# bifurcationkit/BifurcationKit.jl

Measured on AMD Instinct MI355X. Metric: newton_krylov_corrector_steps_per_s, higher is better.
Workload: dtype f64

## Files before the change

### bifurcationkit.jl_amd/_lib.py

```python
from __future__ import annotations

import ctypes as C
import os

_HERE = os.path.dirname(os.path.abspath(__file__))
LIB_PATH = os.environ.get("BKHIP_LIB") or os.path.join(_HERE, "lib", "libbkhip.so")

BK_ABI_VERSION = 6
BK_UNIQUE_ID_BYTES = 128
BK_MAX_PARAMS = 8
BK_MAX_NEWTON_ITER = 64

BK_PDE_SH, BK_PDE_SH1D, BK_PDE_CGL2D = 1, 2, 3
BK_GMRES_KRYLOVKIT, BK_GMRES_ITERATIVESOLVERS, BK_GMRES_KRYLOVJL = 0, 1, 2
BK_KRYLOV_MINRES, BK_KRYLOV_CG = 3, 4

c_double_p = C.POINTER(C.c_double)
c_int_p = C.POINTER(C.c_int)


class ProblemDesc(C.Structure):
    _fields_ = [("pde", C.c_int), ("ndim", C.c_int), ("n", C.c_int * 3), ("l", C.c_double * 3)]


# ... 96 lines not shown
    "bk_prof_enable": (I, [VP, I]),
    "bk_prof_reset": (I, [VP]),
    "bk_prof_get": (I, [VP, C.c_char_p, c_double_p, C.POINTER(C.c_longlong), c_double_p]),
    "bk_solver_history": (I, [VP, c_double_p, SZ, C.POINTER(SZ), I]),
    "bk_solver_block_log": (I, [VP, c_double_p, SZ, C.POINTER(SZ), I]),
    "bk_malloc": (I, [VP, SZ, C.POINTER(VP)]),
    "bk_free": (I, [VP, VP]),
    "bk_upload": (I, [VP, VP, c_double_p, SZ]),
    "bk_download": (I, [VP, c_double_p, VP, SZ]),
    "bk_vec_copy": (I, [VP, SZ, VP, VP]),
    "bk_vec_zero": (I, [VP, SZ, VP]),
    "bk_vec_scale": (I, [VP, SZ, D, VP]),
    "bk_vec_axpby": (I, [VP, SZ, D, VP, D, VP]),
    "bk_vec_dot": (I, [VP, SZ, VP, VP, c_double_p]),
    "bk_vec_nrm2": (I, [VP, SZ, VP, c_double_p]),
    "bk_vec_nrminf": (I, [VP, SZ, VP, c_double_p]),
    "bk_krylov_multidot": (I, [VP, SZ, VP, SZ, I, VP, c_double_p]),
    "bk_krylov_multiaxpy": (I, [VP, SZ, VP, SZ, I, c_double_p, VP, D, VP, c_double_p]),
    "bk_problem_create": (I, [VP, C.POINTER(ProblemDesc), C.POINTER(VP)]),
    "bk_problem_destroy": (I, [VP]),
    "bk_problem_nlocal": (I, [VP, C.POINTER(SZ), c_int_p, c_int_p]),
    "bk_residual": (I, [VP, VP, c_double_p, I, VP]),
    "bk_residual_dparam": (I, [VP, VP, c_double_p, I, I, D, VP]),
    "bk_jacobian": (I, [VP, VP, c_double_p, I, C.POINTER(VP)]),
    "bk_op_destroy": (I, [VP]),
    "bk_jacobian_adjoint": (I, [VP, VP, c_double_p, I, C.POINTER(VP)]),
    "bk_op_apply": (I, [VP, VP, D, D, VP]),
    "bk_precond_sh_create": (I, [VP, D, C.POINTER(VP)]),
    "bk_precond_lap_create": (I, [VP, D, C.POINTER(VP)]),
    "bk_precond_cgl_create": (I, [VP, D, D, C.POINTER(VP)]),
    "bk_precond_destroy": (I, [VP]),
    "bk_precond_apply": (I, [VP, VP, VP]),
    "bk_precond_op_apply": (I, [VP, VP, VP, VP, D, D, VP, c_int_p]),
    "bk_precond_check_norm": (I, [VP, VP, VP, VP, VP, D, D, I, c_double_p, c_int_p]),
    "bk_gmres_default_opts": (None, [C.POINTER(GmresOpts), I]),
    "bk_gmres": (I, [VP, VP, VP, VP, D, D, C.POINTER(GmresOpts), VP, c_int_p, c_int_p, c_double_p]),
    "bk_gmres2": (I, [VP, VP, VP, VP, VP, VP, D, D, C.POINTER(GmresOpts), VP, c_int_p, c_int_p]),
    "bk_palc_update": (I, [VP, SZ, D, VP, VP, VP]),
    "bk_bls_bordering": (I, [VP, VP, VP, VP, D, VP, D, D, D, I, D, D, C.POINTER(BorderingOpts),
                             C.POINTER(GmresOpts), VP, VP, c_double_p, c_int_p, c_int_p]),
    "bk_bls_matrixfree": (I, [VP, VP, VP, VP, D, VP, D, D, D, I, D, D, C.POINTER(GmresOpts), VP, c_double_p,
                              c_int_p, c_int_p]),
    "bk_bls_block_bordering": (I, [VP, VP, I, C.POINTER(VP), C.POINTER(VP), c_double_p, VP, c_double_p,
                                   C.POINTER(GmresOpts), VP, VP, c_double_p, c_int_p, c_int_p]),
    "bk_bls_block_matrixfree": (I, [VP, VP, I, C.POINTER(VP), C.POINTER(VP), c_double_p, VP, c_double_p, I, D, D,
                                    C.POINTER(GmresOpts), VP, c_double_p, c_int_p, c_int_p]),
    "bk_bls_matrixfree_pl": (I, [VP, VP, VP, VP, D, VP, D, D, D, I, D, D, C.POINTER(GmresOpts), VP, VP, c_double_p,
                                 c_int_p, c_int_p]),
    "bk_bls_block_matrixfree_pl": (I, [VP, VP, I, C.POINTER(VP), C.POINTER(VP), c_double_p, VP, c_double_p, I, D, D,
                                       C.POINTER(GmresOpts), VP, VP, c_double_p, c_int_p, c_int_p]),
    "bk_bordered_tail": (I, [VP, SZ, I, VP, VP, C.POINTER(VP), C.POINTER(VP), c_double_p, c_double_p]),
    "bk_gmres_cshift": (I, [VP, VP, VP, VP, VP, VP, D, D, D, C.POINTER(GmresOpts), VP, c_int_p, c_int_p, c_double_p]),
    "bk_bls_bordering_cshift": (I, [VP, VP, VP, VP, VP, VP, D, D, VP, VP, D, D, D, D, D, D, D, C.POINTER(GmresOpts),
                                    VP, VP, VP, c_double_p, c_int_p, c_int_p]),
    "bk_bls_matrixfree_pl_cshift": (I, [VP, VP, VP, VP, VP, VP, D, D, VP, VP, D, D, D, D, D, D, D, C.POINTER(GmresOpts),
                                        VP, VP, VP, c_double_p, c_int_p, c_int_p]),
    "bk_cbordered_tail": (I, [VP, SZ, VP, VP, VP, VP, VP, VP, VP, VP, c_double_p, c_double_p]),
    "bk_eig_shiftinvert": (I, [VP, VP, I, C.POINTER(EigOpts), C.POINTER(GmresOpts), VP, c_double_p, c_double_p,
                               VP, VP, SZ, c_int_p, c_int_p, c_int_p]),
    "bk_eig_set_start_vector": (I, [VP, VP]),
    "bk_eig_krylovkit": (I, [VP, VP, I, C.POINTER(EigOpts), c_double_p, c_double_p, VP, VP, SZ, c_int_p, c_int_p, c_int_p]),
    "bk_newton": (I, [VP, VP, VP, c_double_p, I, C.POINTER(NewtonOpts), C.POINTER(GmresOpts), VP,
                      C.POINTER(NewtonResult)]),
    "bk_cont_create": (I, [VP, VP, c_double_p, I, I, VP, D, VP, D, C.POINTER(ContOpts), C.POINTER(NewtonOpts),
                           C.POINTER(BorderingOpts), C.POINTER(GmresOpts), VP, C.POINTER(EigOpts),
                           C.POINTER(GmresOpts), VP, C.POINTER(ContStepResult), C.POINTER(VP)]),
    "bk_cont_step": (I, [VP, C.POINTER(ContStepResult)]),
    "bk_cont_get": (I, [VP, VP, c_double_p, VP, c_double_p, c_double_p]),
    "bk_cont_destroy": (I, [VP]),
    "bk_cont_clone": (I, [VP, C.POINTER(VP)]),
    "bk_cont_locate_bifurcation": (I, [VP, C.POINTER(BisectionOpts), C.POINTER(BisectionResult)]),
    "bk_newton_deflated": (I, [VP, VP, VP, c_double_p, I, C.POINTER(VP), I, D, D, I, D, C.POINTER(NewtonOpts),
                               C.POINTER(GmresOpts), VP, C.POINTER(NewtonResult)]),
    "bk_deflation_dots": (I, [VP, SZ, VP, VP, C.POINTER(VP), I, c_double_p, c_double_p]),
    "bk_newton_deflated_exact": (I, [VP, VP, VP, c_double_p, I, C.POINTER(VP), I, D, D, I, I, C.POINTER(NewtonOpts),
                                     C.POINTER(GmresOpts), VP, C.POINTER(DeflatedResult)]),
    "bk_deflation_dist": (I, [VP, SZ, VP, C.POINTER(VP), I, c_double_p, c_double_p]),
    "bk_vec_perturb": (I, [VP, SZ, VP, D, C.c_ulonglong, C.c_ulonglong]),
    "bk_defcont_seek": (I, [VP, VP, VP, c_double_p, I, C.POINTER(VP), I, D, D, I, I, I, D, I, C.POINTER(GmresOpts), VP,
                            c_double_p, I, C.POINTER(DefContSeekResult)]),
    "bk_newton_palc": (I, [VP, VP, VP, c_double_p, VP, D, VP, D, D, D, c_double_p, I, I, D, D,
                           C.POINTER(NewtonOpts), C.POINTER(BorderingOpts), C.POINTER(GmresOpts), VP,
                           C.POINTER(NewtonResult)]),
    "bk_d2f": (I, [VP, VP, c_double_p, I, VP, VP, VP]),
    "bk_djdp": (I, [VP, VP, c_double_p, I, I, VP, VP]),
    "bk_fold_contract": (I, [VP, VP, c_double_p, I, I, VP, VP, I, C.POINTER(VP), c_double_p]),
    "bk_fold_border": (I, [VP, VP, c_double_p, I, I, VP, VP, VP, c_double_p]),
    "bk_fold_terms": (I, [VP, VP, VP, c_double_p, I, I, VP, VP, C.POINTER(BorderingOpts), C.POINTER(GmresOpts), VP, VP, VP,
                          c_double_p, c_double_p, c_int_p, c_int_p]),
    "bk_fold_linsolve": (I, [VP, VP, VP, c_double_p, I, I, VP, VP, I, C.POINTER(VP), c_double_p, C.POINTER(GmresOpts), VP,
                             C.POINTER(VP), c_double_p, c_int_p, c_int_p]),
    "bk_newton_fold": (I, [VP, VP, VP, c_double_p, c_double_p, I, I, VP, VP, C.POINTER(NewtonOpts), C.POINTER(BorderingOpts),
                           C.POINTER(GmresOpts), VP, VP, VP, c_double_p, C.POINTER(NewtonResult)]),
    "bk_hopf_d2f": (I, [VP, VP, c_double_p, I, VP, VP, VP]),
    "bk_hopf_djdp": (I, [VP, VP, c_double_p, I, I, VP, VP]),
    "bk_hopf_contract": (I, [VP, VP, c_double_p, I, I, VP, VP, VP, VP, I, C.POINTER(VP), c_double_p]),
    "bk_hopf_terms": (I, [VP, VP, VP, c_double_p, I, I, D, VP, VP, VP, VP, C.POINTER(GmresOpts), VP, VP, VP, VP, VP,
                          c_double_p, c_double_p, c_double_p, c_int_p, c_int_p]),
    "bk_hopf_linsolve": (I, [VP, VP, VP, c_double_p, I, I, VP, VP, VP, VP, I, C.POINTER(VP), c_double_p, C.POINTER(GmresOpts),
                             VP, C.POINTER(VP), c_double_p, c_int_p, c_int_p]),
    "bk_newton_hopf": (I, [VP, VP, VP, c_double_p, c_double_p, c_double_p, I, I, VP, VP, VP, VP, C.POINTER(NewtonOpts),
                           C.POINTER(GmresOpts), VP, VP, VP, VP, VP, c_double_p, C.POINTER(NewtonResult)]),
    "bk_hopf_d3f": (I, [VP, VP, c_double_p, I, VP, VP, VP, VP]),
    "bk_hopf_nf_rhs": (I, [VP, VP, c_double_p, I, VP, VP, VP, VP, VP]),
    "bk_hopf_nf_contract": (I, [VP, VP, c_double_p, I, I, VP, VP, VP, VP, VP, VP, VP, VP, c_double_p]),
    "bk_hopf_normal_form": (I, [VP, VP, VP, c_double_p, I, I, D, VP, VP, VP, VP, C.POINTER(GmresOpts), VP, VP, VP, VP, VP,
                                c_double_p, c_int_p, c_int_p]),
    "bk_hopf_orbit": (I, [VP, SZ, VP, VP, VP, VP, VP, VP, VP, D, D, I, c_double_p, C.POINTER(VP)]),
    "bk_bautin_rhs3": (I, [VP, VP, c_double_p, I, VP, VP, VP, VP, VP, c_double_p, VP, VP, VP, VP]),
    "bk_bautin_rhs4": (I, [VP, VP, c_double_p, I, VP, VP, VP, VP, VP, VP, VP, VP, VP, c_double_p, VP, VP, VP]),
    "bk_bautin_contract": (I, [VP, VP, c_double_p, I, VP, VP, VP, VP, VP, VP, VP, VP, VP, VP, VP, VP, VP, VP, c_double_p]),
    "bk_bautin_normal_form": (I, [VP, VP, VP, c_double_p, I, D, VP, VP, VP, VP, VP, VP, VP, c_double_p, C.POINTER(GmresOpts), VP,
                                  VP, VP, VP, VP, VP, VP, VP, c_double_p, c_int_p, c_int_p]),
    "bk_d3f": (I, [VP, VP, c_double_p, I, VP, VP, VP, VP]),
    "bk_nf1d_dots": (I, [VP, VP, c_double_p, I, I, VP, VP, c_double_p]),
    "bk_nf1d_rhs": (I, [VP, VP, c_double_p, I, I, VP, D, D, VP, VP]),
    "bk_nf1d_contract": (I, [VP, VP, c_double_p, I, I, VP, VP, VP, VP, c_double_p]),
    "bk_nf1d_predict": (I, [VP, SZ, VP, VP, VP, VP, I, c_double_p, c_double_p, c_double_p, C.POINTER(VP)]),
    "bk_normal_form_1d": (I, [VP, VP, VP, c_double_p, I, I, VP, VP, C.POINTER(BorderingOpts), C.POINTER(GmresOpts), VP, VP, VP,
                              c_double_p, c_int_p, c_int_p]),
    "bk_cusp_dots": (I, [VP, VP, c_double_p, I, VP, VP, c_double_p]),
    "bk_cusp_rhs": (I, [VP, VP, c_double_p, I, VP, D, VP]),
    "bk_cusp_contract": (I, [VP, VP, c_double_p, I, VP, VP, VP, c_double_p]),
    "bk_cusp_normal_form": (I, [VP, VP, VP, c_double_p, I, VP, VP, C.POINTER(BorderingOpts), C.POINTER(GmresOpts), VP, VP,
                                c_double_p, c_int_p, c_int_p]),
    "bk_nfnd_dots": (I, [VP, VP, c_double_p, I, I, I, C.POINTER(VP), c_double_p]),
    "bk_nfnd_rhs": (I, [VP, VP, c_double_p, I, I, I, C.POINTER(VP), c_double_p, c_double_p, C.POINTER(VP)]),
    "bk_nfnd_contract": (I, [VP, VP, c_double_p, I, I, I, C.POINTER(VP), VP, C.POINTER(VP), c_double_p]),
    "bk_normal_form_nd": (I, [VP, VP, VP, c_double_p, I, I, I, C.POINTER(VP), C.POINTER(GmresOpts), VP, VP, C.POINTER(VP),
                              c_double_p, c_int_p, c_int_p]),
    "bk_potrap_create": (I, [VP, I, C.POINTER(VP)]),
    "bk_potrap_destroy": (I, [VP]),
    "bk_potrap_set_section": (I, [VP, VP, VP]),
    "bk_potrap_residual": (I, [VP, VP, D, c_double_p, I, VP, c_double_p]),
    "bk_potrap_jvp": (I, [VP, VP, D, c_double_p, I, VP, D, VP, c_double_p]),
    "bk_potrap_op_create": (I, [VP, VP, D, c_double_p, I, C.POINTER(VP)]),
    "bk_potrap_update_section": (I, [VP, VP, D, c_double_p, I]),
    "bk_potrap_dparam": (I, [VP, VP, D, c_double_p, I, I, VP]),
    "bk_precond_potrap_create": (I, [VP, D, D, C.POINTER(VP)]),
    "bk_precond_potrap_set_period": (I, [VP, D]),
    "bk_precond_potrap_transform_paths": (I, [VP, c_int_p]),
    "bk_potrap_get_section": (I, [VP, VP, VP]),
    "bk_potrap_solve": (I, [VP, VP, VP, VP, D, VP, c_double_p, C.POINTER(GmresOpts), C.POINTER(SolveResult)]),
    "bk_potrap_jvp_adjoint": (I, [VP, VP, D, c_double_p, I, VP, D, VP, c_double_p]),
    "bk_potrap_op_adjoint_create": (I, [VP, VP, D, c_double_p, I, C.POINTER(VP)]),
    "bk_precond_potrap_adjoint_create": (I, [VP, D, D, C.POINTER(VP)]),
    "bk_potrap_bordered_solve": (I, [VP, VP, VP, VP, D, VP, D, D, VP, D, D, VP, c_double_p, c_double_p, C.POINTER(GmresOpts),
                                     C.POINTER(SolveResult)]),
    "bk_potrap_fold_border": (I, [VP, VP, D, c_double_p, I, I, VP, D, VP, VP, c_double_p, c_double_p]),
    "bk_potrap_fold_terms": (I, [VP, VP, D, c_double_p, I, VP, D, VP, D, VP, VP, C.POINTER(GmresOpts), VP, c_double_p, VP,
                                 c_double_p, c_double_p, c_int_p, c_int_p]),
    "bk_potrap_fold_linsolve": (I, [VP, VP, D, c_double_p, I, I, VP, D, VP, VP, I, C.POINTER(VP), c_double_p, c_double_p,
                                    C.POINTER(GmresOpts), C.POINTER(VP), c_double_p, c_double_p, c_int_p, c_int_p]),
    "bk_potrap_newton_fold": (I, [VP, VP, c_double_p, c_double_p, c_double_p, I, I, VP, D, VP, D, VP, VP, C.POINTER(NewtonOpts),
                                  C.POINTER(GmresOpts), VP, c_double_p, VP, c_double_p, c_double_p, C.POINTER(NewtonResult),
                                  c_int_p]),
    "bk_potrap_ivp_march": (I, [VP, VP, D, c_double_p, I, VP, VP]),
    "bk_precond_potrap_ivp_create": (I, [VP, D, D, D, C.POINTER(VP)]),
    "bk_precond_potrap_ivp_transform_paths": (I, [VP, c_int_p]),
    "bk_potrap_monodromy_create": (I, [VP, VP, D, c_double_p, I, D, D, C.POINTER(GmresOpts), C.POINTER(VP)]),
    "bk_potrap_monodromy_solve": (I, [VP, VP, VP, c_int_p, c_int_p]),
    "bk_potrap_monodromy_stats": (I, [VP, c_int_p, c_int_p, c_int_p, c_int_p]),
    "bk_eig_krylovkit_lm": (I, [VP, VP, I, C.POINTER(EigOpts), c_double_p, c_double_p, VP, VP, SZ, c_int_p, c_int_p, c_int_p]),
}

_lib = None
# ... 38 lines not shown
```

### bifurcationkit.jl_amd/csrc/common.h

```cpp
#pragma once

#include <hip/hip_runtime.h>
#include <rccl/rccl.h>

#include <cstdarg>
#include <cstdio>
#include <cstring>
#include <map>
#include <set>
#include <string>
#include <utility>
#include <vector>

#include "../../include/bkhip.h"

namespace bk {

constexpr int kMaxBasis = 64;
constexpr int kRedSlots = 256;
constexpr int kRedBlocks = 1024;
constexpr int kPartialVals = 72;
constexpr size_t kPartialDoubles = (size_t)kRedBlocks * kPartialVals;
constexpr double kCancelTol = 1e-8;
constexpr int kRecChunks = 16;
// ... 98 lines not shown
namespace bk {

int set_error(bk_ctx* ctx, const char* fmt, ...);

#define BK_HIP(ctx, call)                                                                     \
    do {                                                                                      \
        hipError_t e_ = (call);                                                               \
        if (e_ != hipSuccess)                                                                 \
            return bk::set_error((ctx), "%s:%d: %s failed: %s", __FILE__, __LINE__, #call,    \
                                 hipGetErrorString(e_));                                      \
    } while (0)

#define BK_NCCL(ctx, call)                                                                    \
    do {                                                                                      \
        ncclResult_t e_ = (call);                                                             \
        if (e_ != ncclSuccess)                                                                \
            return bk::set_error((ctx), "%s:%d: %s failed: %s", __FILE__, __LINE__, #call,    \
                                 ncclGetErrorString(e_));                                     \
    } while (0)

#define BK_TRY(call)             \
    do {                         \
        int s_ = (call);         \
        if (s_ != 0) return s_;  \
    } while (0)

bk_ctx* ctx_lane(bk_ctx* ctx);
void ctx_lane_merge(bk_ctx* ctx, bk_ctx* lane);

int ws_get(bk_ctx* ctx, size_t n, double** out);
void ws_put(bk_ctx* ctx, double* p);

struct WsGuard {
    bk_ctx* ctx;
    std::vector<double*> ptrs;
    explicit WsGuard(bk_ctx* c) : ctx(c) {}
    ~WsGuard() { for (double* p : ptrs) ws_put(ctx, p); }
    int get(size_t n, double** out) {
        int s = ws_get(ctx, n, out);
        if (s == 0) ptrs.push_back(*out);
        return s;
    }
};

struct ProfScope {
    bk_ctx* ctx;
    ProfEntry* e = nullptr;
    hipEvent_t start = nullptr, stop = nullptr;
    ProfScope(bk_ctx* c, const char* name, double alg_bytes);
    ~ProfScope();
};

int reduce_finish(bk_ctx* ctx, int nblocks, int nvals, int op);
int comm_allreduce_host(bk_ctx* ctx, double* buf, int n, int op);
int comm_allreduce_dev(bk_ctx* ctx, hipStream_t stream, double* dbuf, int n, int op);
int ctx_sync(bk_ctx* ctx);
void proxy_destroy(bk_ctx* ctx);

void blas_release(bk_ctx* ctx);
int v_copy(bk_ctx* ctx, size_t n, const double* x, double* y);
int v_zero(bk_ctx* ctx, size_t n, double* x);
int v_scale(bk_ctx* ctx, size_t n, double a, double* x);
int v_axpby(bk_ctx* ctx, size_t n, double a, const double* x, double b, double* y);
int v_axpbyz(bk_ctx* ctx, size_t n, double a, const double* x, double b, const double* y, double* z);
int v_pw_scale(bk_ctx* ctx, size_t n, const double* x, const double* u, double A, double B, double C, double* z);
int v_dot(bk_ctx* ctx, size_t n, const double* x, const double* y, double* out);
int v_dot2(bk_ctx* ctx, size_t n, const double* x, const double* y1, const double* y2, double* out2);
int v_nrm2(bk_ctx* ctx, size_t n, const double* x, double* out);
int v_diff_nrm2(bk_ctx* ctx, size_t n, const double* x, const double* y, double* out);
int v_axpy_dot(bk_ctx* ctx, size_t n, double c, const double* r, double* y, const double* z, double* out);
int v_minres_update(bk_ctx* ctx, size_t n, double cz, const double* z, double c1, const double* w1, double c2, const double* w2,
                    double* w, double phi, double* x);
int v_minres_update2(bk_ctx* ctx, size_t n, double cza, const double* za, double c1a, double c2a, double czb, const double* zb, double c1b,
                     double c2b, const double* m2, const double* m1, double* wa, double* wb, double phia, double phib, double* x);
int v_nrminf(bk_ctx* ctx, size_t n, const double* x, double* out);
int v_multidot(bk_ctx* ctx, size_t n, const double* V, size_t ldv, int k, const double* w, double* out);
bool v_multidot_gram_ok(bk_ctx* ctx, size_t n, const double* V, size_t ldv, int k, const double* w);
int v_multidot_gram(bk_ctx* ctx, size_t n, const double* V, size_t ldv, int k, const double* w, double* out, double* gram);
int v_multiaxpy(bk_ctx* ctx, size_t n, const double* V, size_t ldv, int k, const double* c,
                const double* src, double scale, double* dst, double* nrm2sq);
bool v_block_ok(bk_ctx* ctx, size_t n, const double* V, size_t ldv);
int v_block_dots(bk_ctx* ctx, size_t n, const double* V, size_t ldv, int kold, int r0, int nr, double* D, double* T);
int v_block_axpy(bk_ctx* ctx, size_t n, double* V, size_t ldv, int k, int s, const double* Cm, const double* Tm);
int v_arnoldi_step_dev(bk_ctx* ctx, size_t n, double* V, size_t ldv, int k, const double* w, double eta, double orth_tol,
                       double* rec, double* coef, double* gram = nullptr);
int v_basis_combine(bk_ctx* ctx, size_t n, const double* V, size_t ldv, int m, const double* Qhost, int kout,
                    double* dst, size_t lddst);
int v_fill_random(bk_ctx* ctx, size_t n, size_t global_offset, unsigned long long seed, double* x);

}
```

### bifurcationkit.jl_amd/csrc/cont.hip

```cpp
#include <cmath>
#include <vector>

#include "ops.h"

using namespace bk;

struct bk_cont {
    bk_ctx* ctx = nullptr;
    bk_problem* prob = nullptr;
    size_t n = 0;
    double Nglob = 1.0;
    double params[BK_MAX_PARAMS];
    int nparams = 0, ipar = 0;
    bk_cont_opts co;
    bk_newton_opts no;
    bk_bordering_opts bo;
    bk_gmres_opts lo;
    bk_precond* pl = nullptr;
    bool has_eig = false;
    bk_eig_opts eo;
    bk_gmres_opts elo;
    bk_precond* epl = nullptr;
    double *zu = nullptr, *zoldu = nullptr, *tauu = nullptr, *predu = nullptr, *work = nullptr, *work2 = nullptr;
    double zp = 0, zoldp = 0, taup = 0, predp = 0, ds = 0;
// ... 100 lines not shown
        if (r->vals_re[i] > c->co.tol_stability) {
            ++nu;
            if (std::fabs(r->vals_im[i]) > c->co.tol_stability) ++ni;
        }
    }
    r->nvals = nvals;
    r->eig_converged = nconv >= nev;
    r->eig_numops = nops;
    c->n_unstable_prev = c->n_unstable;
    c->n_imag_prev = c->n_imag;
    c->n_unstable = nu;
    c->n_imag = ni;
    c->nvals = nvals;
    for (int i = 0; i < nvals; ++i) { c->vals_re[i] = r->vals_re[i]; c->vals_im[i] = r->vals_im[i]; }
    return 0;
}

}

extern "C" {

int bk_cont_create(bk_ctx* ctx, bk_problem* prob, const double* params, int nparams, int ipar, const double* u0,
                   double p0, const double* u1, double p1, const bk_cont_opts* copts, const bk_newton_opts* nopts,
                   const bk_bordering_opts* bopts, const bk_gmres_opts* lsopts, bk_precond* pl,
                   const bk_eig_opts* eopts, const bk_gmres_opts* eig_lsopts, bk_precond* eig_pl,
                   bk_cont_step_result* init, bk_cont** out) {
    if (!ctx || !prob || !params || !u0 || !u1 || !copts || !nopts || !bopts || !lsopts || !out) return -1;
    if (ipar < 0 || ipar >= nparams || nparams > BK_MAX_PARAMS) return set_error(ctx, "bad parameter index");
    if (copts->detect && (!eopts || !eig_lsopts)) return set_error(ctx, "bk_cont_create: detect needs eigensolver options");
    if (nopts->max_iterations > BK_MAX_NEWTON_ITER) return set_error(ctx, "max_iterations > %d", BK_MAX_NEWTON_ITER);
    bk_cont* c = new bk_cont();
    c->ctx = ctx; c->prob = prob; c->n = prob->nloc;
    for (int a = 0; a < prob->desc.ndim; ++a) c->Nglob *= prob->desc.n[a];
    if (prob->desc.pde == BK_PDE_CGL2D) c->Nglob *= 2.0;
    for (int i = 0; i < BK_MAX_PARAMS; ++i) c->params[i] = i < nparams ? params[i] : 0.0;
    c->nparams = nparams; c->ipar = ipar;
    c->co = *copts; c->no = *nopts; c->bo = *bopts; c->lo = *lsopts; c->pl = pl;
    c->has_eig = copts->detect != 0;
    if (c->has_eig) { c->eo = *eopts; c->elo = *eig_lsopts; c->epl = eig_pl; }
    c->thick = c->has_eig && ctx->opt("eig_thick_start", 0.0) != 0.0;
    double** bufs[] = {&c->zu, &c->zoldu, &c->tauu, &c->predu, &c->work, &c->work2, &c->eigx0};
    for (double** b : bufs) {
        if (b == &c->eigx0 && !c->thick) continue;
        if (hipMalloc(b, c->n * sizeof(double)) != hipSuccess) {
            bk_cont_destroy(c);
            return set_error(ctx, "bk_cont_create: device allocation failed");
        }
    }
    int s = 0;
    c->ds = copts->ds;
    if ((s = v_copy(ctx, c->n, u0, c->zu)) || (s = v_copy(ctx, c->n, u0, c->zoldu))) { bk_cont_destroy(c); return s; }
    c->zp = c->zoldp = p0;
    bk_cont_step_result r0 = {};
    r0.converged = 1; r0.p = p0; r0.ds_used = c->ds; r0.n_unstable = -1; r0.n_imag = -1;
    if (c->has_eig && (s = eigen(c, &r0))) { bk_cont_destroy(c); return s; }
    r0.n_unstable = c->n_unstable; r0.n_imag = c->n_imag;
    if ((s = secant_tangent(c, u1, p1, u0, p0, c->ds)) || (s = predictor(c))) { bk_cont_destroy(c); return s; }
    r0.ds_next = c->ds;
    if (init) *init = r0;
    *out = c;
    return 0;
}

int bk_cont_destroy(bk_cont* c) {
    if (!c) return 0;
    double* bufs[] = {c->zu, c->zoldu, c->tauu, c->predu, c->work, c->work2, c->eigx0};
    for (double* b : bufs)
        if (b) (void)hipFree(b);
    delete c;
    return 0;
}

int bk_cont_step(bk_cont* c, bk_cont_step_result* r) {
    if (!c || !r) return -1;
    bk_ctx* ctx = c->ctx;
    *r = bk_cont_step_result{};
    r->n_unstable = c->n_unstable; r->n_imag = c->n_imag;
    r->p = c->zp; r->ds_used = c->ds; r->ds_next = c->ds;
    if (c->step > 0 && !(c->zp > c->co.p_min && c->zp < c->co.p_max)) {
        r->stop = 2;
        return 0;
    }
    double* x = c->work;
    BK_TRY(v_copy(ctx, c->n, c->predu, x));
    double p = c->predp;
    bk_newton_result nr = {};
    if (c->predp <= c->co.p_min || c->predp >= c->co.p_max) {
        c->predp = p = std::min(std::max(c->predp, c->co.p_min), c->co.p_max);
        double par[BK_MAX_PARAMS];
        for (int i = 0; i < c->nparams; ++i) par[i] = c->params[i];
        par[c->ipar] = p;
        BK_TRY(bk_newton(ctx, c->prob, x, par, c->nparams, &c->no, &c->lo, c->pl, &nr));
        r->natural = 1;
    } else {
        BK_TRY(bk_newton_palc(ctx, c->prob, x, &p, c->zu, c->zp, c->tauu, c->taup, c->ds, c->co.theta, c->params,
                              c->nparams, c->ipar, c->co.p_min, c->co.p_max, &c->no, &c->bo, &c->lo, c->pl, &nr));
    }
    r->converged = nr.converged; r->itnewton = nr.itnewton; r->itlinear = nr.itlinear;
    c->converged = nr.converged != 0;
    for (int i = 0; i <= nr.itnewton && i <= BK_MAX_NEWTON_ITER; ++i) r->residuals[i] = nr.residuals[i];
    const int prev_unst = c->n_unstable;
    if (nr.converged) {
        BK_TRY(v_copy(ctx, c->n, c->zu, c->zoldu));
        c->zoldp = c->zp;
        BK_TRY(v_copy(ctx, c->n, x, c->zu));
        c->zp = p;
        if (c->has_eig) {
            BK_TRY(eigen(c, r));
            if (prev_unst != -1 && c->n_unstable != prev_unst) r->bifurcation = 1;
        }
        c->step += 1;
    }
    r->p = c->zp;
    r->n_unstable = c->n_unstable; r->n_imag = c->n_imag;
    r->step = c->step;
    double ds = c->ds;
    if (!c->stepsizecontrol) {
    } else if (!nr.converged) {
        if (std::fabs(ds) <= c->co.dsmin) {
            r->stop = 1;
            return 0;
        }
        ds = std::copysign(std::max(std::fabs(ds) / 2.0, c->co.dsmin), ds);
    } else {
        const double Nmax = c->no.max_iterations;
        const double factor = (Nmax - nr.itnewton) / Nmax;
        ds = ds * (1.0 + c->co.a * factor * factor);
    }
    if (c->stepsizecontrol)
        ds = std::copysign(std::min(std::max(std::fabs(ds), c->co.dsmin), c->co.dsmax), ds);
    c->ds = ds;
    r->ds_next = ds;
    if (nr.converged) {
        if (c->co.tangent == 0) {
            BK_TRY(secant_tangent(c, c->zu, c->zp, c->zoldu, c->zoldp, ds));
            r->tangent_converged = 1;
        } else {
            BK_TRY(bordered_tangent(c, &r->tangent_converged));
        }
    }
    BK_TRY(predictor(c));
    return 0;
}

static int cont_copy_state(bk_cont* dst, const bk_cont* src) {
    double* d[] = {dst->zu, dst->zoldu, dst->tauu, dst->predu};
    const double* from[] = {src->zu, src->zoldu, src->tauu, src->predu};
    for (int i = 0; i < 4; ++i) BK_TRY(v_copy(src->ctx, src->n, from[i], d[i]));
    dst->zp = src->zp; dst->zoldp = src->zoldp; dst->taup = src->taup; dst->predp = src->predp; dst->ds = src->ds;
    dst->n_unstable = src->n_unstable; dst->n_imag = src->n_imag; dst->step = src->step;
    dst->n_unstable_prev = src->n_unstable_prev; dst->n_imag_prev = src->n_imag_prev;
    dst->stepsizecontrol = src->stepsizecontrol; dst->converged = src->converged;
    dst->nvals = src->nvals;
    for (int i = 0; i < src->nvals; ++i) { dst->vals_re[i] = src->vals_re[i]; dst->vals_im[i] = src->vals_im[i]; }
    if (src->thick && dst->thick && src->have_x0) BK_TRY(v_copy(src->ctx, src->n, src->eigx0, dst->eigx0));
    dst->have_x0 = src->thick && dst->thick && src->have_x0;
    return 0;
}

int bk_cont_clone(bk_cont* src, bk_cont** out) {
    if (!src || !out) return -1;
    bk_cont* c = new bk_cont(*src);
    c->zu = c->zoldu = c->tauu = c->predu = c->work = c->work2 = c->eigx0 = nullptr;
    double** bufs[] = {&c->zu, &c->zoldu, &c->tauu, &c->predu, &c->work, &c->work2, &c->eigx0};
    for (double** b : bufs) {
        if (b == &c->eigx0 && !c->thick) continue;
        if (hipMalloc(b, c->n * sizeof(double)) != hipSuccess) {
            bk_cont_destroy(c);
            return set_error(src->ctx, "bk_cont_clone: device allocation failed");
        }
    }
    const int s = cont_copy_state(c, src);
    if (s != 0) { bk_cont_destroy(c); return s; }
    *out = c;
    return 0;
}

int bk_cont_locate_bifurcation(bk_cont* c, const bk_bisection_opts* bo, bk_bisection_result* res) {
    if (!c || !bo || !res) return -1;
// ... 193 lines not shown
```

### bifurcationkit.jl_amd/csrc/ops.h

```cpp
#pragma once

#include "common.h"

namespace bk {

int halo_exchange(bk_ctx* ctx, hipStream_t stream, const double* v, size_t plane, int nplanes, int width, double* halo_lo,
                  double* halo_hi);

int comm_alltoallv(bk_ctx* ctx, const double* sendbuf, const size_t* scount, const size_t* sdispl, double* recvbuf,
                   const size_t* rcount, const size_t* rdispl);

struct ShArgs {
    int nx, ny, nz;
    int nzg, zoff;
    double ax, ay, az;
    double l, nu;
    double a0, a1;
    double ag = 0.0;
    bool ag_set = false;
    int mode;
    const double* v;
    const double* u;
    double* out;
    const double* halo_lo;
// ... 93 lines not shown
                     double* out, double* dot, int* fused);
    int dparam(const double* u, const double* params, int nparams, int ipar, double eps, const double* f0, double* out);
};

struct bk_op {
    bk_ctx* ctx = nullptr;
    size_t n = 0;
    int ntail = 0;
    virtual ~bk_op() {}
    virtual int apply(const double* x, const double* xt, double a0, double a1, double* out, double* outt) = 0;
    virtual int apply_axpy_dot(const double* x, double a0, double a1, double c, const double* r, double* out, double* dot);
    virtual bool shift_is_free() const { return false; }
    virtual int apply_block(const double* x, int s, double a0, double a1, const double* theta, double* const* outs) {
        for (int i = 0; i < s; ++i) {
            const int e = apply(i == 0 ? x : outs[i - 1], nullptr, a0 - (theta ? theta[i] : 0.0), a1, outs[i], nullptr);
            if (e != 0) return e;
        }
        return 0;
    }
    virtual int apply_parts(const double* x, double a0, double aL, double ag, double* out) { return 1; }
    virtual const bk_problem* sh_problem() const { return nullptr; }
    virtual bool sh_state(const double** u, double* l, double* nu) const { return false; }
    virtual int apply_check(const double* x, const double* xt, double a0, double a1, double* out, double* outt) {
        return apply(x, xt, a0, a1, out, outt);
    }
    virtual int check_norm(const double* x, double a0, double a1, double* nrm, int* done) { *done = 0; return 0; }
    virtual int apply_check_resume(const double* x, double a0, double a1, double* out) { return apply_check(x, nullptr, a0, a1, out, nullptr); }
    virtual bool hessenberg_shift() const { return false; }
    virtual double monomial_shift() const { return 0.0; }
    virtual double rearranged_origin() const { return 0.0; }
    virtual bool arm_v0(const double* src, double scale, double* dst) { return false; }
    virtual void disarm_v0() {}
};

struct bk_precond {
    bk_ctx* ctx = nullptr;
    size_t n = 0;
    virtual ~bk_precond() {}
    virtual int apply(const double* v, double* out) = 0;
    virtual int apply_dot(const double* v, double* out, double* dot);
    virtual int apply_dot_pre_axpy(double* y, double c, const double* r, double* out, double* dot);
    virtual int apply_nrm2(const double* v, double c, const double* add, double* nrm2_out, bool store_sum = true);
    virtual bool nrm2_spectral_ok() const { return false; }
    virtual bool is_l1_plus_shift(const bk_problem* prob, double* shift) const { return false; }
    virtual int apply_pw(const double* x, const bk::DctFuse& d, double cx, double ct, double* out);
    int pw_src_first(bk::DctFuse& d);
    virtual bool pw_fused_ok(const double* x, const double* u, const double* out) const { return false; }
    virtual int apply_pw_chain(const double* x, const bk::DctFuse& d, int s, const double* cx, double ct, double* const* outs);
    virtual bool pw_plan_ok() const { return false; }
    int pw_agreed = -1;
};

namespace bk {

struct PdeJacobian : bk_op {
    bk_problem* prob;
    const double* u;
    double params[BK_MAX_PARAMS];
    bool adjoint = false;
    int apply(const double* x, const double* xt, double a0, double a1, double* out, double* outt) override;
    int apply_axpy_dot(const double* x, double a0, double a1, double c, const double* r, double* out, double* dot) override;
    bool shift_is_free() const override { return true; }
    int apply_parts(const double* x, double a0, double aL, double ag, double* out) override;
    const bk_problem* sh_problem() const override;
    bool sh_state(const double** u_, double* l, double* nu) const override;
};

bk_precond* precond_lane_shadow(bk_precond* pl, bk_ctx* lane);

struct GmresResult {
    int converged = 0;
    int niter = 0;
    double resnorm = 0.0;
};
int gmres_core(bk_ctx* ctx, bk_op* A, const double* b, const double* bt, double* x, double* xt, double alpha0,
               double alpha1, const bk_gmres_opts& o, GmresResult* res);
int linsolve(bk_ctx* ctx, bk_op* J, const double* rhs, double* x, double a0, double a1, const bk_gmres_opts& o,
             bk_precond* pl, GmresResult* res);
int linsolve2(bk_ctx* ctx, bk_op* J, const double* rhs1, double* x1, const double* rhs2, double* x2, double a0, double a1,
              const bk_gmres_opts& o, bk_precond* pl, GmresResult* r1, GmresResult* r2);
int bls_bordering(bk_ctx* ctx, bk_op* J, const double* dR, const double* dzu, double dzp, const double* R, double nn,
                  double xiu, double xip, bool has_shift, double shift, double dotscale, const bk_bordering_opts& bo,
                  const bk_gmres_opts& ls, bk_precond* pl, double* dX, double* dl, int* converged, int itlinear[2],
                  double* xnew = nullptr);
struct PrecOpView {
    bk_op* op = nullptr;
    bool tmode = false;
    double alpha0 = 0.0, alpha1 = 1.0;
};
int prec_op_create(bk_ctx* ctx, bk_op* J, bk_precond* pl, double a0, double a1, int order, double* tmp, PrecOpView* out);
int bls_matrixfree_pl(bk_ctx* ctx, bk_op* J, int m, const double* const* a, const double* const* b, double bscale, const double* c,
                      const double* rhst, const double* rhsb, bool has_shift, double shift, const bk_gmres_opts& ls, bk_precond* pl,
                      double* u1, double* u2, GmresResult* res, const double* const* atil = nullptr);
int cshift_op_create(bk_ctx* ctx, bk_op* J, bk_precond* pl, double a0r, double a0i, double a1, int order, double* tmp, bk_op** out);
int bordered_tail(bk_ctx* ctx, size_t n, int m, double* y, const double* x, const double* const* atil, const double* const* b,
                  const double* coef, double* dots);
int cbordered_tail(bk_ctx* ctx, size_t n, double* yr, double* yi, const double* xr, const double* xi, const double* atr,
                   const double* ati, const double* br, const double* bi, const double* coef, double* dots);
int bls_matrixfree_pl_cshift(bk_ctx* ctx, bk_op* J, const double* const a[2], const double* const b[2], double bscale, const double c[2],
                             const double* const rhst[2], const double rhsb[2], const double shift[2], const bk_gmres_opts& ls,
                             bk_precond* pl, double* u1_re, double* u1_im, double u2[2], GmresResult* res);
int newton_cb(const bk_newton_opts* no, const double* x, const double* fx, double residual, int step, int itlinear, double p,
              const double* z0u, double z0p, int from_newton);

}
```

### bifurcationkit.jl_amd/csrc/solver.hip

```cpp
#include <cmath>
#include <cstdio>
#include <thread>
#include <vector>

#include "dense.h"
#include "ops.h"
#include "sstep.h"
#include "stream.h"

namespace bk {

namespace {

constexpr double kCheckSpectralDefault = 1.0;

constexpr double kMonomialShiftDefault = 0.0;

inline size_t round_up(size_t n, size_t m) { return (n + m - 1) / m * m; }

struct Basis {
    double* V = nullptr;
    size_t ld = 0;
    int nt = 0;
    double dlt = 0.0;
// ... 1007 lines not shown
        o->dim = 30; o->maxiter = 100; o->atol = 1e-12; o->rtol = 1e-12;
    }
}

int bk_gmres(bk_ctx* ctx, bk_op* J, const double* rhs, double* x, double a0, double a1, const bk_gmres_opts* opts,
             bk_precond* pl, int* converged, int* niter, double* resnorm) {
    if (!ctx || !J || !rhs || !x || !opts) return -1;
    GmresResult r;
    BK_TRY(linsolve(ctx, J, rhs, x, a0, a1, *opts, pl, &r));
    if (converged) *converged = r.converged;
    if (niter) *niter = r.niter;
    if (resnorm) *resnorm = r.resnorm;
    return 0;
}

int bk_precond_op_apply(bk_ctx* ctx, bk_precond* pl, bk_op* J, const double* x, double a0, double a1, double* out, int* stencil_free) {
    if (!ctx || !pl || !J || !x || !out) return -1;
    if (J->ntail != 0) return set_error(ctx, "bk_precond_op_apply: operator must be unbordered");
    if (out == x) return set_error(ctx, "bk_precond_op_apply: out must not alias x");
    WsGuard ws(ctx);
    ShiftPrecOp W;
    W.ctx = ctx; W.n = J->n; W.ntail = 0;
    W.J = J; W.P = pl; W.a0 = a0; W.a1 = a1; W.order = 0; W.tmp = nullptr;
    BK_TRY(W.init_fold());
    BK_TRY(ws.get(J->n, &W.tmp));
    if (stencil_free) *stencil_free = W.tmode ? 1 : 0;
    return W.tmode ? W.apply(x, nullptr, W.t_alpha0, W.t_alpha1, out, nullptr) : W.apply(x, nullptr, 0.0, 1.0, out, nullptr);
}

int bk_precond_check_norm(bk_ctx* ctx, bk_precond* pl, bk_op* J, const double* x, const double* rhs, double a0, double a1, int flavor,
                          double* nrm, int* spectral) {
    if (!ctx || !pl || !J || !x || !rhs || !nrm) return -1;
    if (J->ntail != 0) return set_error(ctx, "bk_precond_check_norm: operator must be unbordered");
    if (flavor != BK_GMRES_KRYLOVKIT && flavor != BK_GMRES_ITERATIVESOLVERS && flavor != BK_GMRES_KRYLOVJL)
        return set_error(ctx, "bk_precond_check_norm: a GMRES flavor");
    WsGuard ws(ctx);
    ShiftPrecOp W;
    W.ctx = ctx; W.n = J->n; W.ntail = 0;
    W.J = J; W.P = pl; W.a0 = a0; W.a1 = a1; W.order = flavor == BK_GMRES_KRYLOVKIT ? 0 : 1; W.tmp = nullptr;
    BK_TRY(W.init_fold());
    W.rhs = rhs;
    BK_TRY(ws.get(J->n, &W.tmp));
    const double alpha0 = W.tmode ? W.t_alpha0 : 0.0, alpha1 = W.tmode ? W.t_alpha1 : 1.0;
    int have = 0;
    BK_TRY(W.check_norm(x, alpha0, alpha1, nrm, &have));
    if (spectral) *spectral = have;
    if (have) return 0;
    double *b = nullptr, *w = nullptr;
    BK_TRY(ws.get(J->n, &b));
    BK_TRY(ws.get(J->n, &w));
    BK_TRY(pl->apply(rhs, b));
    BK_TRY(W.apply_check(x, nullptr, alpha0, alpha1, w, nullptr));
    return v_diff_nrm2(ctx, J->n, b, w, nrm);
}

int bk_abi_version(void) { return BK_ABI_VERSION; }

int bk_gmres2(bk_ctx* ctx, bk_op* J, const double* rhs1, const double* rhs2, double* x1, double* x2, double a0,
              double a1, const bk_gmres_opts* opts, bk_precond* pl, int* converged, int niter[2]) {
    if (!ctx || !J || !rhs1 || !rhs2 || !x1 || !x2 || !opts) return -1;
    if (x1 == x2) return set_error(ctx, "bk_gmres2: x1 and x2 must be distinct buffers");
    GmresResult r1, r2;
    BK_TRY(linsolve2(ctx, J, rhs1, x1, rhs2, x2, a0, a1, *opts, pl, &r1, &r2));
    if (converged) *converged = r1.converged & r2.converged;
    if (niter) { niter[0] = r1.niter; niter[1] = r2.niter; }
    return 0;
}

}

namespace bk {

struct BorderingState {
    double* dx = nullptr;
    bool have_dx = false;
    int it_dx = 0;
    int cv_dx = 1;
};

namespace {

template <int VEC, bool NTH>
__global__ void __launch_bounds__(kThreads) palc_update_kernel(size_t n, double a, const double* __restrict__ dx,
                                                               const double* __restrict__ x1, double* x, int has_dx) {
    auto one = [&](double d, double v, double xv) {
        double t = 0.0;
        if (has_dx) t = __dmul_rn(a, d);
        t = __dadd_rn(t, v);
        return __dadd_rn(-t, xv);
    };
    if (VEC == 2) {
        stream_loop<4>(n >> 1, [&](auto uc, size_t i0, size_t st) {
            constexpr int UU = decltype(uc)::value;
            double2 dv[UU], vv[UU], xv[UU];
#pragma unroll
            for (int u = 0; u < UU; ++u) {
                dv[u] = ld2<NTH>(dx, i0 + u * st);
                vv[u] = ld2<NTH>(x1, i0 + u * st);
                xv[u] = ld2<NTH>(x, i0 + u * st);
            }
#pragma unroll
            for (int u = 0; u < UU; ++u) {
                const double rx = one(dv[u].x, vv[u].x, xv[u].x), ry = one(dv[u].y, vv[u].y, xv[u].y);
                if (NTH) {
                    nt_d2 r; r.x = rx; r.y = ry;
                    __builtin_nontemporal_store(r, reinterpret_cast<nt_d2*>(x) + (i0 + u * st));
                } else {
                    reinterpret_cast<double2*>(x)[i0 + u * st] = make_double2(rx, ry);
                }
            }
        });
        if ((n & 1) && blockIdx.x == 0 && threadIdx.x == 0) x[n - 1] = one(dx[n - 1], x1[n - 1], x[n - 1]);
    } else {
        for (size_t i = (size_t)blockIdx.x * kThreads + threadIdx.x; i < n; i += (size_t)gridDim.x * kThreads) x[i] = one(dx[i], x1[i], x[i]);
    }
}

}

int palc_update(bk_ctx* ctx, size_t n, double dl, const double* dx, const double* x1, double* x) {
    if (n == 0) return 0;
    ProfScope ps(ctx, "blas1", 32.0 * n);
    const bool vec = aligned16(dx) && aligned16(x1) && aligned16(x);
    const int grid = grid_for(n, vec ? 2 : 1, 4096);
    const double a = -dl;
    const int has_dx = a != 0.0 ? 1 : 0;
    if (vec && nt_hint(ctx, n))
        hipLaunchKernelGGL((palc_update_kernel<2, true>), dim3(grid), dim3(kThreads), 0, ctx->stream, n, a, dx, x1, x, has_dx);
    else if (vec)
        hipLaunchKernelGGL((palc_update_kernel<2, false>), dim3(grid), dim3(kThreads), 0, ctx->stream, n, a, dx, x1, x, has_dx);
    else
        hipLaunchKernelGGL((palc_update_kernel<1, false>), dim3(grid), dim3(kThreads), 0, ctx->stream, n, a, dx, x1, x, has_dx);
    BK_HIP(ctx, hipGetLastError());
    return 0;
}

static int bec(bk_ctx* ctx, bk_op* J, const double* dR, const double* dzu, double dzp, const double* R, double nn,
               double xiu, double xip, bool has_shift, double shift, double dotscale, const bk_gmres_opts& ls,
               bk_precond* pl, BorderingState& st, double* x1, double* dl, int* cv, int it[2], double* xnew = nullptr) {
    const size_t n = J->n;
    GmresResult r1;
    const double a0 = has_shift ? shift : 0.0;
    if (!st.have_dx) {
        GmresResult r2;
        BK_TRY(linsolve2(ctx, J, R, x1, dR, st.dx, a0, 1.0, ls, pl, &r1, &r2));
        st.have_dx = true; st.it_dx = r2.niter; st.cv_dx = r2.converged;
    } else {
        BK_TRY(linsolve(ctx, J, R, x1, a0, 1.0, ls, pl, &r1));
    }
    double d[2];
    BK_TRY(v_dot2(ctx, n, dzu, x1, st.dx, d));
    d[0] *= dotscale; d[1] *= dotscale;
    *dl = (nn - d[0] * xiu) / (dzp * xip - d[1] * xiu);
    if (xnew) BK_TRY(palc_update(ctx, n, *dl, st.dx, x1, xnew));
    else BK_TRY(v_axpby(ctx, n, -(*dl), st.dx, 1.0, x1));
    *cv = r1.converged & st.cv_dx;
    it[0] = r1.niter; it[1] = st.it_dx;
    return 0;
}

int bls_bordering(bk_ctx* ctx, bk_op* J, const double* dR, const double* dzu, double dzp, const double* R, double nn,
                  double xiu, double xip, bool has_shift, double shift, double dotscale, const bk_bordering_opts& bo,
                  const bk_gmres_opts& ls, bk_precond* pl, double* dX, double* dl, int* converged, int itlinear[2],
                  double* xnew) {
    if (xnew && bo.check_precision) return set_error(ctx, "bls_bordering: the fused update needs check_precision off");
    const size_t n = J->n;
    WsGuard ws(ctx);
    BorderingState st;
    BK_TRY(ws.get(n, &st.dx));
    int cv = 0, it[2] = {0, 0};
    BK_TRY(bec(ctx, J, dR, dzu, dzp, R, nn, xiu, xip, has_shift, shift, dotscale, ls, pl, st, dX, dl, &cv, it, xnew));
    int k = 0;
    bool fail = true;
    double *dXr = nullptr, *dX1 = nullptr;
    while (bo.check_precision && k < bo.k && fail) {
        if (!dXr) { BK_TRY(ws.get(n, &dXr)); BK_TRY(ws.get(n, &dX1)); }
        BK_TRY(J->apply(dX, nullptr, has_shift ? shift : 0.0, 1.0, dXr, nullptr));
        BK_TRY(v_axpby(ctx, n, *dl, dR, 1.0, dXr));
        BK_TRY(v_axpby(ctx, n, 1.0, R, -1.0, dXr));
        double dd, nr;
        BK_TRY(v_dot(ctx, n, dzu, dX, &dd));
        const double dlr = nn - xip * dzp * (*dl) - xiu * dotscale * dd;
        BK_TRY(v_nrm2(ctx, n, dXr, &nr));
        fail = nr > bo.tol || std::fabs(dlr) > bo.tol;
        if (fail) {
            double dl1 = 0.0;
            BK_TRY(bec(ctx, J, dR, dzu, dzp, dXr, dlr, xiu, xip, has_shift, shift, dotscale, ls, pl, st, dX1, &dl1, &cv, it));
            BK_TRY(v_axpby(ctx, n, 1.0, dX1, 1.0, dX));
            *dl += dl1;
            k += 1;
        }
    }
    if (converged) *converged = cv;
    if (itlinear) { itlinear[0] = it[0]; itlinear[1] = it[1]; }
    return 0;
}

struct BorderedMapOp : bk_op {
    bk_op* J;
    const double* a[BK_MAX_BORDER];
    const double* bvec[BK_MAX_BORDER];
    double bscale;
    double c[BK_MAX_BORDER * BK_MAX_BORDER];
    bool has_shift;
    double shift;
    int apply(const double* x, const double* xt, double b0, double b1, double* out, double* outt) override {
        const int m = ntail;
        BK_TRY(J->apply(x, nullptr, b0 + b1 * (has_shift ? shift : 0.0), b1, out, nullptr));
        for (int i = 0; i < m; ++i)
            if (xt[i] != 0.0 && b1 != 0.0) BK_TRY(v_axpby(ctx, n, b1 * xt[i], a[i], 1.0, out));
        for (int i = 0; i < m; ++i) {
            double d;
            BK_TRY(v_dot(ctx, n, bvec[i], x, &d));
            double cx = 0.0;
            for (int j = 0; j < m; ++j) cx += c[i * m + j] * xt[j];
            outt[i] = b0 * xt[i] + b1 * (bscale * d + cx);
        }
        return 0;
    }
};

int bls_matrixfree(bk_ctx* ctx, bk_op* J, const double* dR, const double* dzu, double dzp, const double* R, double n, double xiu,
                   double xip, bool has_shift, double shift, double dotscale, const bk_gmres_opts& ls, double* dX, double* dl,
                   int* converged, int* itlinear) {
    if (ls.flavor >= BK_KRYLOV_MINRES) return set_error(ctx, "bk_bls_matrixfree: the bordered operator is not symmetric (use a GMRES flavor)");
    BorderedMapOp M;
    M.ctx = ctx; M.n = J->n; M.ntail = 1;
    M.J = J; M.a[0] = dR; M.bvec[0] = dzu; M.bscale = xiu * dotscale; M.c[0] = dzp * xip;
    M.has_shift = has_shift; M.shift = shift;
    GmresResult r;
    BK_TRY(gmres_core(ctx, &M, R, &n, dX, dl, 0.0, 1.0, ls, &r));
    if (converged) *converged = r.converged;
    if (itlinear) *itlinear = r.niter;
    return 0;
}

}

extern "C" {

int bk_bls_bordering(bk_ctx* ctx, bk_op* J, const double* dR, const double* dzu, double dzp, const double* R,
                     double n, double xiu, double xip, int has_shift, double shift, double dotscale,
                     const bk_bordering_opts* bopts, const bk_gmres_opts* lsopts, bk_precond* pl, double* dX,
                     double* dl, int* converged, int itlinear[2]) {
    if (!ctx || !J || !dR || !dzu || !R || !bopts || !lsopts || !dX || !dl) return -1;
    if (dX == R || dX == dR || dX == dzu) return set_error(ctx, "bk_bls_bordering: dX must be a fresh buffer");
    if (bopts->k < 1) return set_error(ctx, "BorderingBLS: number of recursions must be positive");
    return bls_bordering(ctx, J, dR, dzu, dzp, R, n, xiu, xip, has_shift != 0, shift, dotscale, *bopts, *lsopts, pl, dX,
                         dl, converged, itlinear);
}

int bk_palc_update(bk_ctx* ctx, size_t n, double dl, const double* dx, const double* x1, double* x) {
    if (!ctx || !dx || !x1 || !x) return -1;
    if (x == dx || x == x1) return set_error(ctx, "bk_palc_update: x must not alias dx or x1");
    return palc_update(ctx, n, dl, dx, x1, x);
}

int bk_bls_matrixfree(bk_ctx* ctx, bk_op* J, const double* dR, const double* dzu, double dzp, const double* R,
                      double n, double xiu, double xip, int has_shift, double shift, double dotscale,
                      const bk_gmres_opts* lsopts, double* dX, double* dl, int* converged, int* itlinear) {
    if (!ctx || !J || !dR || !dzu || !R || !lsopts || !dX || !dl) return -1;
    if (dX == R || dX == dR || dX == dzu) return set_error(ctx, "bk_bls_matrixfree: dX must be a fresh buffer");
    return bls_matrixfree(ctx, J, dR, dzu, dzp, R, n, xiu, xip, has_shift != 0, shift, dotscale, *lsopts, dX, dl, converged, itlinear);
}

int bk_bls_block_bordering(bk_ctx* ctx, bk_op* J, int m, const double* const* b, const double* const* c, const double* d,
                           const double* rhst, const double* rhsb, const bk_gmres_opts* lsopts, bk_precond* pl,
                           double* u1, double* u2, int* converged, int* itlinear) {
    if (!ctx || !J || !b || !c || !d || !rhst || !rhsb || !lsopts || !u1 || !u2) return -1;
    if (m < 1 || m > BK_MAX_BORDER) return set_error(ctx, "Linear bordered solver, wrong sizes! (1 <= m <= %d)", BK_MAX_BORDER);
    if (u1 == rhst) return set_error(ctx, "bk_bls_block_bordering: u1 must be a fresh buffer");
    const size_t n = J->n;
    WsGuard ws(ctx);
    double* x2[BK_MAX_BORDER];
    GmresResult g;
    BK_TRY(linsolve(ctx, J, rhst, u1, 0.0, 1.0, *lsopts, pl, &g));
    int cv = 1;
    for (int j = 0; j < m; ++j) {
        if (!b[j] || !c[j]) return -1;
        BK_TRY(ws.get(n, &x2[j]));
        BK_TRY(linsolve(ctx, J, b[j], x2[j], 0.0, 1.0, *lsopts, pl, &g));
        cv &= g.converged;
        if (itlinear) itlinear[j] = g.niter;
    }
    double S[BK_MAX_BORDER][BK_MAX_BORDER + 1];
    for (int i = 0; i < m; ++i) {
        double t;
        for (int j = 0; j < m; ++j) {
            BK_TRY(v_dot(ctx, n, c[i], x2[j], &t));
            S[i][j] = d[i * m + j] - t;
        }
        BK_TRY(v_dot(ctx, n, c[i], u1, &t));
        S[i][m] = rhsb[i] - t;
    }
    for (int k = 0; k < m; ++k) {
        int piv = k;
        for (int i = k + 1; i < m; ++i)
            if (std::fabs(S[i][k]) > std::fabs(S[piv][k])) piv = i;
        if (S[piv][k] == 0.0) return set_error(ctx, "bk_bls_block_bordering: singular Schur complement");
        if (piv != k)
            for (int j = 0; j <= m; ++j) std::swap(S[k][j], S[piv][j]);
        for (int i = k + 1; i < m; ++i) {
            const double f = S[i][k] / S[k][k];
            for (int j = k; j <= m; ++j) S[i][j] -= f * S[k][j];
        }
    }
    for (int i = m - 1; i >= 0; --i) {
        double t = S[i][m];
        for (int j = i + 1; j < m; ++j) t -= S[i][j] * u2[j];
        u2[i] = t / S[i][i];
    }
    for (int j = 0; j < m; ++j) BK_TRY(v_axpby(ctx, n, -u2[j], x2[j], 1.0, u1));
    if (converged) *converged = cv;
    return 0;
}

int bk_bls_block_matrixfree(bk_ctx* ctx, bk_op* J, int m, const double* const* a, const double* const* b, const double* c,
                            const double* rhst, const double* rhsb, int has_shift, double shift, double dotscale,
                            const bk_gmres_opts* lsopts, double* u1, double* u2, int* converged, int* itlinear) {
    if (!ctx || !J || !a || !b || !c || !rhst || !rhsb || !lsopts || !u1 || !u2) return -1;
    if (m < 1 || m > BK_MAX_BORDER) return set_error(ctx, "Linear bordered solver, wrong sizes! (1 <= m <= %d)", BK_MAX_BORDER);
    if (u1 == rhst) return set_error(ctx, "bk_bls_block_matrixfree: u1 must be a fresh buffer");
    if (lsopts->flavor >= BK_KRYLOV_MINRES) return set_error(ctx, "bk_bls_block_matrixfree: the bordered operator is not symmetric (use a GMRES flavor)");
    BorderedMapOp M;
    M.ctx = ctx; M.n = J->n; M.ntail = m;
    M.J = J; M.bscale = dotscale;
    for (int i = 0; i < m; ++i) {
        if (!a[i] || !b[i]) return -1;
        M.a[i] = a[i]; M.bvec[i] = b[i];
        for (int j = 0; j < m; ++j) M.c[i * m + j] = c[i * m + j];
    }
    M.has_shift = has_shift != 0; M.shift = shift;
    GmresResult r;
    BK_TRY(gmres_core(ctx, &M, rhst, rhsb, u1, u2, 0.0, 1.0, *lsopts, &r));
    if (converged) *converged = r.converged;
    if (itlinear) *itlinear = r.niter;
    return 0;
}

}

namespace bk {

static int norm_of(bk_ctx* ctx, size_t n, const double* x, bool inf, double* out) {
    return inf ? v_nrminf(ctx, n, x, out) : v_nrm2(ctx, n, x, out);
}

int newton_cb(const bk_newton_opts* no, const double* x, const double* fx, double residual, int step, int itlinear,
              double p, const double* z0u, double z0p, int from_newton) {
    if (no->max_residual > 0.0 && !(residual < no->max_residual)) return 0;
    if (no->callback) return no->callback(no->callback_user, x, fx, residual, step, itlinear, p, z0u, z0p, from_newton) != 0;
    return 1;
}

}

extern "C" {

int bk_newton(bk_ctx* ctx, bk_problem* prob, double* x, const double* params, int nparams, const bk_newton_opts* no,
              const bk_gmres_opts* lsopts, bk_precond* pl, bk_newton_result* res) {
    if (!ctx || !prob || !x || !params || !no || !lsopts || !res) return -1;
    if (no->max_iterations > BK_MAX_NEWTON_ITER) return set_error(ctx, "max_iterations > %d", BK_MAX_NEWTON_ITER);
    const size_t n = prob->nloc;
    WsGuard ws(ctx);
    double *fx = nullptr, *u = nullptr;
    BK_TRY(ws.get(n, &fx));
    BK_TRY(ws.get(n, &u));
    BK_TRY(bk_residual(prob, x, params, nparams, fx));
    double r;
    BK_TRY(norm_of(ctx, n, fx, no->norm_inf != 0, &r));
    int step = 0, itlin = 0;
    res->residuals[0] = r;
    int compute = newton_cb(no, x, fx, r, 0, 0, NAN, nullptr, NAN, 1);
    while (step < no->max_iterations && r > no->tol && compute) {
        bk_op* J = nullptr;
        BK_TRY(bk_jacobian(prob, x, params, nparams, &J));
        GmresResult g;
        int s = linsolve(ctx, J, fx, u, 0.0, 1.0, *lsopts, pl, &g);
        bk_op_destroy(J);
        if (s != 0) return s;
        itlin += g.niter;
        BK_TRY(v_axpby(ctx, n, -1.0, u, 1.0, x));
        BK_TRY(bk_residual(prob, x, params, nparams, fx));
        BK_TRY(norm_of(ctx, n, fx, no->norm_inf != 0, &r));
        step += 1;
        res->residuals[step] = r;
        compute = newton_cb(no, x, fx, r, step, g.niter, NAN, nullptr, NAN, 1);
    }
    res->converged = (res->residuals[step] < no->tol) & newton_cb(no, x, fx, r, step, 0, NAN, nullptr, NAN, 1);
    res->itnewton = step;
    res->itlinear = itlin;
    return 0;
}

int bk_newton_palc(bk_ctx* ctx, bk_problem* prob, double* x, double* p, const double* z0u, double z0p,
                   const double* tauu, double taup, double ds, double theta, const double* params, int nparams,
                   int ipar, double p_min, double p_max, const bk_newton_opts* no, const bk_bordering_opts* bo,
                   const bk_gmres_opts* lsopts, bk_precond* pl, bk_newton_result* res) {
    if (!ctx || !prob || !x || !p || !z0u || !tauu || !params || !no || !bo || !lsopts || !res) return -1;
    if (ipar < 0 || ipar >= nparams || nparams > BK_MAX_PARAMS) return set_error(ctx, "bad parameter index");
    if (no->max_iterations > BK_MAX_NEWTON_ITER) return set_error(ctx, "max_iterations > %d", BK_MAX_NEWTON_ITER);
    const size_t n = prob->nloc;
    double Nglob = 1.0;
    for (int a = 0; a < prob->desc.ndim; ++a) Nglob *= prob->desc.n[a];
    if (prob->desc.pde == BK_PDE_CGL2D) Nglob *= 2.0;
    const double dotscale = 1.0 / Nglob;
    const double eps = 1.4901161193847656e-08;
    WsGuard ws(ctx);
    double *res_f = nullptr, *dFdp = nullptr, *u = nullptr, *x_pred = nullptr;
    BK_TRY(ws.get(n, &res_f));
    BK_TRY(ws.get(n, &dFdp));
    BK_TRY(ws.get(n, &u));
    const bool linesearch = no->linesearch != 0;
    if (linesearch) BK_TRY(ws.get(n, &x_pred));
    const double alpha0 = no->alpha > 0.0 ? no->alpha : 1.0;
    const double alpha_min = no->alpha_min > 0.0 ? no->alpha_min : 1e-3;
    double alpha = alpha0;
    double par[BK_MAX_PARAMS];
    for (int i = 0; i < nparams; ++i) par[i] = params[i];
    const bool inf = no->norm_inf != 0;
    double dz0;
    BK_TRY(v_dot(ctx, n, z0u, tauu, &dz0));
    auto Nfun = [&](const double* xx, double pp, double* out) -> int {
        double d;
        BK_TRY(v_dot(ctx, n, xx, tauu, &d));
        *out = (d * dotscale * theta + (pp - z0p) * taup * (1.0 - theta) - ds) - (dz0 * dotscale * theta);
        return 0;
    };
    double pc = *p;
    par[ipar] = pc;
    BK_TRY(bk_residual(prob, x, par, nparams, res_f));
    double res_n, rf;
    BK_TRY(Nfun(x, pc, &res_n));
    BK_TRY(norm_of(ctx, n, res_f, inf, &rf));
    double r = std::max(rf, std::fabs(res_n));
    int step = 0, itlin = 0;
    res->residuals[0] = r;
    bool line_step = true;
    const bool fuse_update = bo->kind == 0 && bo->check_precision == 0 && !linesearch && ctx->opt("palc_fuse_update", 1.0) != 0.0;
    int compute = newton_cb(no, x, res_f, r, 0, 0, pc, z0u, z0p, 0);
    while (step < no->max_iterations && r > no->tol && line_step && compute) {
        par[ipar] = pc;
        BK_TRY(prob->dparam(x, par, nparams, ipar, eps, res_f, dFdp));
        bk_op* J = nullptr;
        BK_TRY(bk_jacobian(prob, x, par, nparams, &J));
        double up = 0.0;
        int cv = 0, it[2] = {0, 0};
        int s;
        if (bo->kind == 1) {
            int itm = 0;
            s = bls_matrixfree(ctx, J, dFdp, tauu, taup, res_f, res_n, theta, 1.0 - theta, false, 0.0, dotscale, *lsopts, u, &up, &cv, &itm);
            it[0] = itm; it[1] = 0;
        } else {
            s = bls_bordering(ctx, J, dFdp, tauu, taup, res_f, res_n, theta, 1.0 - theta, false, 0.0, dotscale, *bo,
                              *lsopts, pl, u, &up, &cv, it, fuse_update ? x : nullptr);
        }
        bk_op_destroy(J);
        if (s != 0) return s;
        itlin += it[0] + it[1];
        if (linesearch) {
            line_step = false;
            while (!line_step && alpha > alpha_min) {
                BK_TRY(v_axpbyz(ctx, n, 1.0, x, -alpha, u, x_pred));
                const double p_pred = pc - alpha * up;
                par[ipar] = p_pred;
                BK_TRY(bk_residual(prob, x_pred, par, nparams, res_f));
                BK_TRY(Nfun(x_pred, p_pred, &res_n));
                BK_TRY(norm_of(ctx, n, res_f, inf, &rf));
                r = std::max(rf, std::fabs(res_n));
                if (r < res->residuals[step]) {
                    if (r < res->residuals[step] / 4.0 && alpha < 1.0) alpha *= 2.0;
                    line_step = true;
                    BK_TRY(v_copy(ctx, n, x_pred, x));
                    pc = std::min(std::max(p_pred, p_min), p_max);
                } else {
                    alpha /= 2.0;
                }
            }
            alpha = alpha0;
            par[ipar] = pc;
        } else {
            if (!fuse_update) BK_TRY(v_axpby(ctx, n, -1.0, u, 1.0, x));
            pc = std::min(std::max(pc - up, p_min), p_max);
            par[ipar] = pc;
            BK_TRY(bk_residual(prob, x, par, nparams, res_f));
            BK_TRY(Nfun(x, pc, &res_n));
            BK_TRY(norm_of(ctx, n, res_f, inf, &rf));
            r = std::max(rf, std::fabs(res_n));
        }
        step += 1;
        res->residuals[step] = r;
        compute = newton_cb(no, x, res_f, r, step, it[0] + it[1], pc, z0u, z0p, 0);
    }
    *p = pc;
    res->converged = (res->residuals[step] < no->tol) & newton_cb(no, x, res_f, r, step, 0, pc, z0u, z0p, 0);
    res->itnewton = step;
    res->itlinear = itlin;
    return 0;
}

}
```

### bifurcationkit.jl_amd/csrc/vecops.hip

```cpp
#include <algorithm>
#include <type_traits>

#include "common.h"
#include "sstep.h"
#include "stream.h"

namespace bk {

namespace {

struct StreamRange { size_t lo, hi, step; };
__device__ __forceinline__ StreamRange stream_range(size_t n2, unsigned xcd) {
    StreamRange r;
    if (xcd) {
        const size_t x = blockIdx.x & 7u, lb = blockIdx.x >> 3, nb = gridDim.x >> 3;
        const size_t per = ((n2 + 7) / 8 + kThreads - 1) / kThreads * kThreads;
        const size_t b0 = x * per < n2 ? x * per : n2, b1 = (x + 1) * per < n2 ? (x + 1) * per : n2;
        r.lo = b0 + lb * kThreads + threadIdx.x; r.hi = b1; r.step = nb * kThreads;
    } else {
        r.lo = (size_t)blockIdx.x * kThreads + threadIdx.x; r.hi = n2; r.step = (size_t)gridDim.x * kThreads;
    }
    return r;
}

inline unsigned xcd_map(bk_ctx* ctx, size_t n, int grid, bool axpy, int k) {
    const int mode = (int)ctx->opt("vec_xcd_map", 1.0);
    if (!(nt_hint(ctx, n) && grid >= 8 && grid % 8 == 0) || mode == 0) return 0u;
    return (mode >= 2 || (axpy && k >= 12)) ? 1u : 0u;
}

__device__ __forceinline__ double max_nan(double a, double b) { return (a != a || a > b) ? a : b; }
__device__ __forceinline__ double wave_max(double v) {
#pragma unroll
    for (int off = 32; off > 0; off >>= 1) v = max_nan(v, __shfl_down(v, off, 64));
    return v;
}

__device__ __forceinline__ void st2nt(double* p, size_t i, double2 v) {
    nt_d2 r; r.x = v.x; r.y = v.y;
    __builtin_nontemporal_store(r, reinterpret_cast<nt_d2*>(p) + i);
}


template <int VEC, bool NTH = false>
__global__ void __launch_bounds__(kThreads) axpbyz_kernel(size_t n, double a, const double* __restrict__ x, double b,
                                                          const double* y, double* z, int has_x, int has_y) {
    const size_t stride = (size_t)gridDim.x * kThreads;
    if (VEC == 2) {
        const size_t n2 = n >> 1;
        auto run = [&](auto hx, auto hy) {
            constexpr bool HX = decltype(hx)::value, HY = decltype(hy)::value;
            stream_loop<4>(n2, [&](auto uc, size_t i0, size_t st) {
                constexpr int UU = decltype(uc)::value;
                double2 xv[UU], yv[UU];
#pragma unroll
                for (int u = 0; u < UU; ++u) {
                    if (HX) xv[u] = ld2<NTH>(x, i0 + u * st);
                    if (HY) yv[u] = ld2<NTH>(y, i0 + u * st);
                }
#pragma unroll
                for (int u = 0; u < UU; ++u) {
                    double2 r = make_double2(0.0, 0.0);
                    if (HX) { r.x = a * xv[u].x; r.y = a * xv[u].y; }
                    if (HY) { r.x += b * yv[u].x; r.y += b * yv[u].y; }
                    if (NTH) st2nt(z, i0 + u * st, r);
                    else reinterpret_cast<double2*>(z)[i0 + u * st] = r;
                }
            });
        };
        if (has_x && has_y) run(std::true_type{}, std::true_type{});
        else if (has_x) run(std::true_type{}, std::false_type{});
        else if (has_y) run(std::false_type{}, std::true_type{});
        else run(std::false_type{}, std::false_type{});
        if ((n & 1) && blockIdx.x == 0 && threadIdx.x == 0) {
            const size_t i = n - 1;
            double r = 0.0;
            if (has_x) r = a * x[i];
            if (has_y) r += b * y[i];
            z[i] = r;
        }
    } else {
        for (size_t i = (size_t)blockIdx.x * kThreads + threadIdx.x; i < n; i += stride) {
            double r = 0.0;
            if (has_x) r = a * x[i];
            if (has_y) r += b * y[i];
// ... 115 lines not shown
            stream_loop<2>(n2, [&](auto uc, size_t i0, size_t st) {
                constexpr int UU = decltype(uc)::value;
                double2 yv[UU], rv[UU], zv[UU];
#pragma unroll
                for (int u = 0; u < UU; ++u) {
                    yv[u] = ld2<NTH>(y, i0 + u * st);
                    if (HR) rv[u] = ld2<NTH>(r, i0 + u * st);
                    zv[u] = ld2<NTH>(z, i0 + u * st);
                }
#pragma unroll
                for (int u = 0; u < UU; ++u) {
                    if (HR) {
                        yv[u].x = fma(c, rv[u].x, yv[u].x); yv[u].y = fma(c, rv[u].y, yv[u].y);
                        if (NTH) st2nt(y, i0 + u * st, yv[u]);
                        else reinterpret_cast<double2*>(y)[i0 + u * st] = yv[u];
                    }
                    s = fma(zv[u].x, yv[u].x, s); s = fma(zv[u].y, yv[u].y, s);
                }
            });
        };
        if (has_r) run(std::true_type{}); else run(std::false_type{});
        if ((n & 1) && blockIdx.x == 0 && threadIdx.x == 0) {
            double yv = y[n - 1];
            if (has_r) { yv = fma(c, r[n - 1], yv); y[n - 1] = yv; }
            s = fma(z[n - 1], yv, s);
        }
    } else {
        for (size_t i = (size_t)blockIdx.x * kThreads + threadIdx.x; i < n; i += stride) {
            double yv = y[i];
            if (has_r) { yv = fma(c, r[i], yv); y[i] = yv; }
            s = fma(z[i], yv, s);
        }
    }
    __shared__ double sm[4];
    s = wave_sum(s);
    if ((threadIdx.x & 63) == 0) sm[threadIdx.x >> 6] = s;
    __syncthreads();
    if (threadIdx.x == 0) partials[blockIdx.x] = (sm[0] + sm[1]) + (sm[2] + sm[3]);
}

template <int VEC, bool NTH = false>
__global__ void __launch_bounds__(kThreads) minres_update_kernel(size_t n, double cz, const double* __restrict__ z, double c1,
                                                                 const double* __restrict__ w1, double c2,
                                                                 const double* __restrict__ w2, double* __restrict__ w,
                                                                 double phi, double* __restrict__ x) {
    const size_t stride = (size_t)gridDim.x * kThreads;
    if (VEC == 2) {
        const size_t n2 = n >> 1;
        stream_loop<2>(n2, [&](auto uc, size_t i0, size_t st) {
            constexpr int UU = decltype(uc)::value;
            double2 zv[UU], a[UU], b[UU], xv[UU];
#pragma unroll
            for (int u = 0; u < UU; ++u) {
                zv[u] = ld2<NTH>(z, i0 + u * st);
                a[u] = ld2<NTH>(w1, i0 + u * st);
                b[u] = ld2<NTH>(w2, i0 + u * st);
                xv[u] = ld2<NTH>(x, i0 + u * st);
            }
#pragma unroll
            for (int u = 0; u < UU; ++u) {
                double2 wv;
                wv.x = fma(c2, b[u].x, fma(c1, a[u].x, cz * zv[u].x));
                wv.y = fma(c2, b[u].y, fma(c1, a[u].y, cz * zv[u].y));
                xv[u].x = fma(phi, wv.x, xv[u].x); xv[u].y = fma(phi, wv.y, xv[u].y);
                if (NTH) { st2nt(w, i0 + u * st, wv); st2nt(x, i0 + u * st, xv[u]); }
                else { reinterpret_cast<double2*>(w)[i0 + u * st] = wv; reinterpret_cast<double2*>(x)[i0 + u * st] = xv[u]; }
            }
        });
        if ((n & 1) && blockIdx.x == 0 && threadIdx.x == 0) {
            const size_t i = n - 1;
            const double wv = fma(c2, w2[i], fma(c1, w1[i], cz * z[i]));
            w[i] = wv;
            x[i] = fma(phi, wv, x[i]);
        }
    } else {
        for (size_t i = (size_t)blockIdx.x * kThreads + threadIdx.x; i < n; i += stride) {
            const double wv = fma(c2, w2[i], fma(c1, w1[i], cz * z[i]));
            w[i] = wv;
            x[i] = fma(phi, wv, x[i]);
        }
    }
}

__global__ void __launch_bounds__(kThreads) absmax_kernel(size_t n, const double* __restrict__ x,
                                                          double* __restrict__ partials) {
    const size_t stride = (size_t)gridDim.x * kThreads;
    double m = 0.0;
    for (size_t i = (size_t)blockIdx.x * kThreads + threadIdx.x; i < n; i += stride) m = max_nan(m, fabs(x[i]));
    __shared__ double sm[4];
    m = wave_max(m);
    if ((threadIdx.x & 63) == 0) sm[threadIdx.x >> 6] = m;
    __syncthreads();
    if (threadIdx.x == 0) partials[blockIdx.x] = max_nan(max_nan(sm[0], sm[1]), max_nan(sm[2], sm[3]));
}

template <int KB, int VEC, bool LDNT = false>
__global__ void __launch_bounds__(kThreads) multidot_kernel(size_t n, const double* __restrict__ V, size_t ldv, int k,
                                                            const double* __restrict__ w,
                                                            double* __restrict__ partials, const double* gate = nullptr,
                                                            unsigned xcd = 0) {
    if (gate && gate[0] == 0.0) return;
    double acc[KB];
#pragma unroll
    for (int j = 0; j < KB; ++j) acc[j] = 0.0;
    double ww = 0.0;
    const size_t stride = (size_t)gridDim.x * kThreads;
    if (VEC == 2) {
        const StreamRange rg = stream_range(n >> 1, xcd);
        for (size_t i = rg.lo; i < rg.hi; i += rg.step) {
            const double2 wv = ld2<LDNT>(w, i);
            ww = fma(wv.x, wv.x, ww); ww = fma(wv.y, wv.y, ww);
#pragma unroll
            for (int j = 0; j < KB; ++j) {
                if (j < k) {
                    const double2 vv = ld2<LDNT>(V + (size_t)j * ldv, i);
                    acc[j] = fma(vv.x, wv.x, acc[j]);
                    acc[j] = fma(vv.y, wv.y, acc[j]);
                }
            }
        }
        if ((n & 1) && blockIdx.x == 0 && threadIdx.x == 0) {
            const double wv = w[n - 1];
            ww = fma(wv, wv, ww);
#pragma unroll
            for (int j = 0; j < KB; ++j)
                if (j < k) acc[j] = fma(V[(size_t)j * ldv + n - 1], wv, acc[j]);
        }
    } else {
        for (size_t i = (size_t)blockIdx.x * kThreads + threadIdx.x; i < n; i += stride) {
            const double wv = w[i];
            ww = fma(wv, wv, ww);
#pragma unroll
            for (int j = 0; j < KB; ++j)
                if (j < k) acc[j] = fma(V[(size_t)j * ldv + i], wv, acc[j]);
        }
    }
    __shared__ double sm[4][KB + 1];
    const int lane = threadIdx.x & 63, wid = threadIdx.x >> 6;
#pragma unroll
    for (int j = 0; j < KB; ++j) {
        const double s = wave_sum(acc[j]);
        if (lane == 0) sm[wid][j] = s;
    }
    {
        const double s = wave_sum(ww);
        if (lane == 0) sm[wid][KB] = s;
    }
    __syncthreads();
    for (int j = threadIdx.x; j <= k; j += kThreads) {
        const int src = (j == k) ? KB : j;
        partials[(size_t)blockIdx.x * (k + 1) + j] = (sm[0][src] + sm[1][src]) + (sm[2][src] + sm[3][src]);
    }
}

template <int KB, int VEC, bool NT = false, bool LDNT = false, int U = 1, bool DEV = false>
__global__ void __launch_bounds__(kThreads) multiaxpy_kernel(size_t n, const double* __restrict__ V, size_t ldv, int k,
                                                             Coefs cf, const double* src, double scale, double* dst,
                                                             int want_norm, double* __restrict__ partials, unsigned xcd = 0,
                                                             const double* __restrict__ dcoef = nullptr, int gated = 0) {
    if (DEV) {
        if (gated && dcoef[kMaxBasis + 1] == 0.0) return;
        scale = dcoef[kMaxBasis];
#pragma unroll
        for (int j = 0; j < KB; ++j) cf.c[j] = j < k ? dcoef[j] : 0.0;
    }
    double nn = 0.0;
    if (VEC == 2) {
        const StreamRange rg = stream_range(n >> 1, xcd);
        const size_t n2 = rg.hi, stride = rg.step;
        for (size_t i0 = rg.lo; i0 < n2; i0 += stride * U) {
            double2 r[U];
// ... 125 lines not shown
    }
    {
        const double s_ = wave_sum(ww);
        if (lane == 0) sm[wid][KB] = s_;
    }
    if (GRAM) {
#pragma unroll
        for (int j = 0; j < KB; ++j) {
            const double s_ = wave_sum(accg[j]);
            if (lane == 0) sm[wid][KB + 1 + j] = s_;
        }
    }
    __syncthreads();
    const int nv = GRAM ? 2 * k + 1 : k + 1;
    for (int j = threadIdx.x; j < nv; j += kThreads) {
        const int src = j < k ? j : (j == k ? KB : KB + 1 + (j - k - 1));
        partials[(size_t)blockIdx.x * nv + j] = (sm[0][src] + sm[1][src]) + (sm[2][src] + sm[3][src]);
    }
}

template <int KB, int U, bool NT, bool LDNT, bool DEV>
__global__ void __launch_bounds__(kThreads) multiaxpy_c_kernel(size_t n, const double* __restrict__ V, size_t ldv, int k, Coefs cf,
                                                               const double* src, double scale, double* dst, int want_norm,
                                                               double* __restrict__ partials,
                                                               const double* __restrict__ dcoef, int gated, int stag) {
    if (DEV) {
        if (gated && dcoef[kMaxBasis + 1] == 0.0) return;
        scale = dcoef[kMaxBasis];
#pragma unroll
        for (int j = 0; j < KB; ++j) cf.c[j] = j < k ? dcoef[j] : 0.0;
    }
    if (stag > 0) {
        const int P = stag & 255, map = (stag >> 8) & 255, units = stag >> 16;
        const int ph = (map == 0 ? (int)(blockIdx.x >> 3) : (int)(blockIdx.x >> 8)) % P;
        const int nburst = ((k + 2) * ph) / P;
        for (int i = 0; i < nburst * units; ++i) __builtin_amdgcn_s_sleep(1);
    }
    double nn = 0.0;
    stream_loop<U>(n >> 1, [&](auto uc, size_t i0, size_t st) {
        constexpr int UU = decltype(uc)::value;
        double2 r[UU];
#pragma unroll
        for (int u = 0; u < UU; ++u) r[u] = src ? ld2<LDNT>(src, i0 + u * st) : make_double2(0.0, 0.0);
#pragma unroll
        for (int j = 0; j < KB; ++j) {
            if (j < k) {
                double2 vv[UU];
#pragma unroll
                for (int u = 0; u < UU; ++u) vv[u] = ld2<LDNT>(V + (size_t)j * ldv, i0 + u * st);
#pragma unroll
                for (int u = 0; u < UU; ++u) { r[u].x = fma(cf.c[j], vv[u].x, r[u].x); r[u].y = fma(cf.c[j], vv[u].y, r[u].y); }
            }
        }
#pragma unroll
        for (int u = 0; u < UU; ++u) {
            r[u].x *= scale; r[u].y *= scale;
            if (NT) st2nt(dst, i0 + u * st, r[u]);
            else reinterpret_cast<double2*>(dst)[i0 + u * st] = r[u];
            nn = fma(r[u].x, r[u].x, nn); nn = fma(r[u].y, r[u].y, nn);
        }
    });
    if ((n & 1) && blockIdx.x == 0 && threadIdx.x == 0) {
        const size_t i = n - 1;
        double r = src ? src[i] : 0.0;
#pragma unroll
        for (int j = 0; j < KB; ++j)
            if (j < k) r = fma(cf.c[j], V[(size_t)j * ldv + i], r);
        r *= scale;
        dst[i] = r;
        nn = fma(r, r, nn);
    }
    if (want_norm) {
        __shared__ double sm[4];
        nn = wave_sum(nn);
        if ((threadIdx.x & 63) == 0) sm[threadIdx.x >> 6] = nn;
        __syncthreads();
        if (threadIdx.x == 0) partials[blockIdx.x] = (sm[0] + sm[1]) + (sm[2] + sm[3]);
    }
}

template <int KB, bool TRI, int U, bool LDNT, int NRT = sstep::kR>
__global__ void __launch_bounds__(kThreads) block_dots_kernel(size_t n, const double* __restrict__ V, size_t ldv, int kb,
                                                              const double* __restrict__ Rv, int nr, double* __restrict__ partials) {
    constexpr int NR = NRT, NT3 = TRI ? NRT * (NRT + 1) / 2 : 1;
    double acc[KB > 0 ? KB : 1][NR], tri[NT3];
#pragma unroll
    for (int i = 0; i < (KB > 0 ? KB : 1); ++i)
#pragma unroll
        for (int r = 0; r < NR; ++r) acc[i][r] = 0.0;
#pragma unroll
    for (int t = 0; t < NT3; ++t) tri[t] = 0.0;
    stream_loop<U>(n >> 1, [&](auto uc, size_t i0, size_t st) {
        constexpr int UU = decltype(uc)::value;
        double2 rv[NR][UU];
#pragma unroll
        for (int r = 0; r < NR; ++r) {
            if (r < nr) {
#pragma unroll
                for (int u = 0; u < UU; ++u) rv[r][u] = ld2<LDNT>(Rv + (size_t)r * ldv, i0 + u * st);
            } else {
#pragma unroll
                for (int u = 0; u < UU; ++u) rv[r][u] = make_double2(0.0, 0.0);
            }
        }
        if (TRI) {
#pragma unroll
            for (int r = 0; r < NR; ++r)
#pragma unroll
                for (int c = r; c < NR; ++c) {
                    double a = tri[TRI ? r * NR - r * (r - 1) / 2 + (c - r) : 0];
#pragma unroll
                    for (int u = 0; u < UU; ++u) { a = fma(rv[r][u].x, rv[c][u].x, a); a = fma(rv[r][u].y, rv[c][u].y, a); }
                    tri[TRI ? r * NR - r * (r - 1) / 2 + (c - r) : 0] = a;
                }
        }
#pragma unroll
        for (int i = 0; i < KB; ++i) {
            if (i < kb) {
                double2 vv[UU];
#pragma unroll
                for (int u = 0; u < UU; ++u) vv[u] = ld2<LDNT>(V + (size_t)i * ldv, i0 + u * st);
#pragma unroll
                for (int r = 0; r < NR; ++r)
#pragma unroll
                    for (int u = 0; u < UU; ++u) { acc[i][r] = fma(vv[u].x, rv[r][u].x, acc[i][r]); acc[i][r] = fma(vv[u].y, rv[r][u].y, acc[i][r]); }
            }
        }
    });
    if ((n & 1) && blockIdx.x == 0 && threadIdx.x == 0) {
        double rl[NR];
#pragma unroll
        for (int r = 0; r < NR; ++r) rl[r] = r < nr ? Rv[(size_t)r * ldv + n - 1] : 0.0;
        if (TRI) {
#pragma unroll
            for (int r = 0; r < NR; ++r)
#pragma unroll
                for (int c = r; c < NR; ++c) tri[TRI ? r * NR - r * (r - 1) / 2 + (c - r) : 0] = fma(rl[r], rl[c], tri[TRI ? r * NR - r * (r - 1) / 2 + (c - r) : 0]);
        }
#pragma unroll
        for (int i = 0; i < KB; ++i)
            if (i < kb) {
                const double vl = V[(size_t)i * ldv + n - 1];
#pragma unroll
                for (int r = 0; r < NR; ++r) acc[i][r] = fma(vl, rl[r], acc[i][r]);
            }
    }
    constexpr int NV = KB * NR + (TRI ? NR * (NR + 1) / 2 : 0);
    __shared__ double sm[4][NV];
    const int lane = threadIdx.x & 63, wid = threadIdx.x >> 6;
#pragma unroll
    for (int i = 0; i < KB; ++i)
#pragma unroll
        for (int r = 0; r < NR; ++r) {
            const double s_ = wave_sum(acc[i][r]);
            if (lane == 0) sm[wid][i * NR + r] = s_;
        }
    if (TRI) {
#pragma unroll
        for (int t = 0; t < NT3; ++t) {
            const double s_ = wave_sum(tri[t]);
            if (lane == 0) sm[wid][KB * NR + t] = s_;
        }
    }
    __syncthreads();
    for (int j = threadIdx.x; j < NV; j += kThreads)
        partials[(size_t)blockIdx.x * NV + j] = (sm[0][j] + sm[1][j]) + (sm[2][j] + sm[3][j]);
}

struct BlockCoefs {
    double c[32][sstep::kS];
    double t[sstep::kS][sstep::kS];
};
template <int KB, int U, bool LDNT>
__global__ void __launch_bounds__(kThreads) block_axpy_kernel(size_t n, const double* V, size_t ldv, int k, double* Pv, int s,
                                                              BlockCoefs cf) {
    constexpr int S = sstep::kS;
    stream_loop<U>(n >> 1, [&](auto uc, size_t i0, size_t st) {
        constexpr int UU = decltype(uc)::value;
        double2 acc[S][UU];
#pragma unroll
        for (int q = 0; q < S; ++q)
#pragma unroll
            for (int u = 0; u < UU; ++u) acc[q][u] = make_double2(0.0, 0.0);
#pragma unroll
        for (int r = 0; r < S; ++r) {
            if (r < s) {
                double2 pv[UU];
#pragma unroll
                for (int u = 0; u < UU; ++u) pv[u] = ld2<LDNT>(Pv + (size_t)r * ldv, i0 + u * st);
#pragma unroll
                for (int q = r; q < S; ++q)
#pragma unroll
                    for (int u = 0; u < UU; ++u) { acc[q][u].x = fma(cf.t[r][q], pv[u].x, acc[q][u].x); acc[q][u].y = fma(cf.t[r][q], pv[u].y, acc[q][u].y); }
            }
        }
#pragma unroll
        for (int i = 0; i < KB; ++i) {
            if (i < k) {
                double2 vv[UU];
#pragma unroll
                for (int u = 0; u < UU; ++u) vv[u] = ld2<LDNT>(V + (size_t)i * ldv, i0 + u * st);
#pragma unroll
                for (int q = 0; q < S; ++q)
#pragma unroll
                    for (int u = 0; u < UU; ++u) { acc[q][u].x = fma(cf.c[i][q], vv[u].x, acc[q][u].x); acc[q][u].y = fma(cf.c[i][q], vv[u].y, acc[q][u].y); }
            }
        }
#pragma unroll
        for (int q = 0; q < S; ++q) {
            if (q < s) {
#pragma unroll
                for (int u = 0; u < UU; ++u) {
                    if (LDNT) st2nt(Pv + (size_t)q * ldv, i0 + u * st, acc[q][u]);
                    else reinterpret_cast<double2*>(Pv + (size_t)q * ldv)[i0 + u * st] = acc[q][u];
                }
            }
        }
    });
    if ((n & 1) && blockIdx.x == 0 && threadIdx.x == 0) {
        const size_t e = n - 1;
        double pl[S], o[S];
        for (int r = 0; r < S; ++r) pl[r] = r < s ? Pv[(size_t)r * ldv + e] : 0.0;
        for (int q = 0; q < S; ++q) {
            double v = 0.0;
            for (int r = 0; r <= q; ++r) v = fma(cf.t[r][q], pl[r], v);
            for (int i = 0; i < k && i < KB; ++i) v = fma(cf.c[i][q], V[(size_t)i * ldv + e], v);
            o[q] = v;
        }
        for (int q = 0; q < s; ++q) Pv[(size_t)q * ldv + e] = o[q];
    }
}

__global__ void __launch_bounds__(256) reduce_stage2_dev(const double* __restrict__ partials, int nblocks, int nvals,
                                                         double* __restrict__ out, const double* gate) {
    if (gate && gate[0] == 0.0) return;
    const int v = blockIdx.x;
    double acc = 0.0;
    for (int b = threadIdx.x; b < nblocks; b += 256) acc += partials[(size_t)b * nvals + v];
    for (int off = 32; off > 0; off >>= 1) acc += __shfl_down(acc, off, 64);
    __shared__ double sm[4];
    if ((threadIdx.x & 63) == 0) sm[threadIdx.x >> 6] = acc;
    __syncthreads();
    if (threadIdx.x == 0) {
        double r = sm[0];
        for (int w = 1; w < 4; ++w) r += sm[w];
        out[v] = r;
    }
}

// ... 190 lines not shown
}

int v_nrm2(bk_ctx* ctx, size_t n, const double* x, double* out) {
    double s = 0.0;
    BK_TRY(dot_launch(ctx, n, x, x, nullptr, 1, &s));
    *out = sqrt(s);
    return 0;
}

int v_axpy_dot(bk_ctx* ctx, size_t n, double c, const double* r, double* y, const double* z, double* out) {
    const int has_r = (r != nullptr && c != 0.0) ? 1 : 0;
    const bool vec = aligned16(y) && aligned16(z) && (!has_r || aligned16(r));
    const int grid = grid_for(n, vec ? 2 : 1, kRedBlocks);
    {
        ProfScope ps(ctx, "blas1", 8.0 * n * (2 + 2 * has_r));
        if (vec && nt_hint(ctx, n)) hipLaunchKernelGGL((axpy_dot_kernel<2, true>), dim3(grid), dim3(kThreads), 0, ctx->stream, n, c, r, has_r, y, z, ctx->d_partials);
        else if (vec) hipLaunchKernelGGL((axpy_dot_kernel<2>), dim3(grid), dim3(kThreads), 0, ctx->stream, n, c, r, has_r, y, z, ctx->d_partials);
        else hipLaunchKernelGGL((axpy_dot_kernel<1>), dim3(grid), dim3(kThreads), 0, ctx->stream, n, c, r, has_r, y, z, ctx->d_partials);
        BK_HIP(ctx, hipGetLastError());
    }
    BK_TRY(reduce_finish(ctx, grid, 1, 0));
    *out = ctx->h_red[0];
    return 0;
}

int v_minres_update(bk_ctx* ctx, size_t n, double cz, const double* z, double c1, const double* w1, double c2, const double* w2,
                    double* w, double phi, double* x) {
    const bool vec = aligned16(z) && aligned16(w1) && aligned16(w2) && aligned16(w) && aligned16(x);
    const int grid = grid_for(n, vec ? 2 : 1, 4096);
    ProfScope ps(ctx, "blas1", 8.0 * n * 6);
    if (vec && nt_hint(ctx, n)) hipLaunchKernelGGL((minres_update_kernel<2, true>), dim3(grid), dim3(kThreads), 0, ctx->stream, n, cz, z, c1, w1, c2, w2, w, phi, x);
    else if (vec) hipLaunchKernelGGL((minres_update_kernel<2>), dim3(grid), dim3(kThreads), 0, ctx->stream, n, cz, z, c1, w1, c2, w2, w, phi, x);
    else hipLaunchKernelGGL((minres_update_kernel<1>), dim3(grid), dim3(kThreads), 0, ctx->stream, n, cz, z, c1, w1, c2, w2, w, phi, x);
    BK_HIP(ctx, hipGetLastError());
    return 0;
}

template <bool NTH>
__global__ void __launch_bounds__(kThreads) minres_update2_kernel(size_t n2, double cza, const double* __restrict__ za, double c1a, double c2a,
                                                                  double czb, const double* __restrict__ zb, double c1b, double c2b,
                                                                  const double* m2, const double* __restrict__ m1, double* __restrict__ wa,
                                                                  double* wb, double phia, double phib, double* __restrict__ x) {
    stream_loop<2>(n2, [&](auto uc, size_t i0, size_t st) {
        constexpr int UU = decltype(uc)::value;
        double2 av[UU], bv[UU], p2[UU], p1[UU], xv[UU];
#pragma unroll
        for (int u = 0; u < UU; ++u) {
            av[u] = ld2<NTH>(za, i0 + u * st);
            bv[u] = ld2<NTH>(zb, i0 + u * st);
            p2[u] = ld2<NTH>(m2, i0 + u * st);
            p1[u] = ld2<NTH>(m1, i0 + u * st);
            xv[u] = ld2<NTH>(x, i0 + u * st);
        }
#pragma unroll
        for (int u = 0; u < UU; ++u) {
            double2 a_, b_;
            a_.x = fma(c2a, p1[u].x, fma(c1a, p2[u].x, cza * av[u].x));
            a_.y = fma(c2a, p1[u].y, fma(c1a, p2[u].y, cza * av[u].y));
            b_.x = fma(c2b, a_.x, fma(c1b, p1[u].x, czb * bv[u].x));
            b_.y = fma(c2b, a_.y, fma(c1b, p1[u].y, czb * bv[u].y));
            xv[u].x = fma(phib, b_.x, fma(phia, a_.x, xv[u].x));
            xv[u].y = fma(phib, b_.y, fma(phia, a_.y, xv[u].y));
            if (NTH) { st2nt(wa, i0 + u * st, a_); st2nt(wb, i0 + u * st, b_); st2nt(x, i0 + u * st, xv[u]); }
            else {
                reinterpret_cast<double2*>(wa)[i0 + u * st] = a_; reinterpret_cast<double2*>(wb)[i0 + u * st] = b_;
                reinterpret_cast<double2*>(x)[i0 + u * st] = xv[u];
            }
        }
    });
}

int v_minres_update2(bk_ctx* ctx, size_t n, double cza, const double* za, double c1a, double c2a, double czb, const double* zb, double c1b,
                     double c2b, const double* m2, const double* m1, double* wa, double* wb, double phia, double phib, double* x) {
    if ((n & 1) || !(aligned16(za) && aligned16(zb) && aligned16(m2) && aligned16(m1) && aligned16(wa) && aligned16(wb) && aligned16(x))) return 1;
    const int grid = grid_for(n, 2, 4096);
    ProfScope ps(ctx, "blas1", 8.0 * n * 8);
    if (nt_hint(ctx, n)) hipLaunchKernelGGL((minres_update2_kernel<true>), dim3(grid), dim3(kThreads), 0, ctx->stream, n >> 1, cza, za, c1a, c2a, czb, zb, c1b, c2b, m2, m1, wa, wb, phia, phib, x);
    else hipLaunchKernelGGL((minres_update2_kernel<false>), dim3(grid), dim3(kThreads), 0, ctx->stream, n >> 1, cza, za, c1a, c2a, czb, zb, c1b, c2b, m2, m1, wa, wb, phia, phib, x);
    BK_HIP(ctx, hipGetLastError());
    return 0;
}

int v_nrminf(bk_ctx* ctx, size_t n, const double* x, double* out) {
    const int grid = grid_for(n, 1, kRedBlocks);
    {
        ProfScope ps(ctx, "blas1", 8.0 * n);
        hipLaunchKernelGGL(absmax_kernel, dim3(grid), dim3(kThreads), 0, ctx->stream, n, x, ctx->d_partials);
        BK_HIP(ctx, hipGetLastError());
    }
    BK_TRY(reduce_finish(ctx, grid, 1, 1));
    *out = ctx->h_red[0];
    return 0;
}

constexpr int kBurstMax = 32;
static bool burst_ok(bk_ctx* ctx, bool vec, size_t n, int k) {
    return vec && k >= 1 && k <= kBurstMax && nt_hint(ctx, n) && ctx->opt("krylov_burst", 1.0) != 0.0;
}
static int burst_grid(bk_ctx* ctx, size_t n, const char* key) {
    return grid_for(n, 2, std::min(kRedBlocks, std::max(8, (int)ctx->opt(key, 512.0))));
}
static void launch_multidot_burst(bk_ctx* ctx, int grid, size_t n, const double* V, size_t ldv, int k, const double* w, const double* gate) {
    const bool u8 = k >= 6 && ctx->opt("dot_burst", 0.0) != 4.0;
#define BK_MDC(KB)                                                                                                                                  \
    do {                                                                                                                                           \
        if (u8) hipLaunchKernelGGL((multidot_c_kernel<KB, 8, true>), dim3(grid), dim3(kThreads), 0, ctx->stream, n, V, ldv, k, w, ctx->d_partials, gate); \
        else hipLaunchKernelGGL((multidot_c_kernel<KB, 4, true>), dim3(grid), dim3(kThreads), 0, ctx->stream, n, V, ldv, k, w, ctx->d_partials, gate);    \
    } while (0)
    if (k <= 4) BK_MDC(4);
    else if (k <= 8) BK_MDC(8);
    else if (k <= 16) BK_MDC(16);
    else if (k <= 24) BK_MDC(24);
    else BK_MDC(32);
#undef BK_MDC
}
static void launch_multidot_gram(bk_ctx* ctx, int grid, size_t n, const double* V, size_t ldv, int k, const double* w, const double* gate,
                                 const double* vn = nullptr) {
    const bool nt = nt_hint(ctx, n);
#define BK_MDG(KB, UU)                                                                                                                              \
    do {                                                                                                                                           \
        if (nt) hipLaunchKernelGGL((multidot_c_kernel<KB, UU, true, true>), dim3(grid), dim3(kThreads), 0, ctx->stream, n, V, ldv, k, w, ctx->d_partials, gate, vn); \
        else hipLaunchKernelGGL((multidot_c_kernel<KB, 4, false, true>), dim3(grid), dim3(kThreads), 0, ctx->stream, n, V, ldv, k, w, ctx->d_partials, gate, vn);    \
    } while (0)
    if (k <= 4) BK_MDG(4, 4);
    else if (k < 6) BK_MDG(8, 4);
    else if (k <= 8) BK_MDG(8, 8);
    else if (k <= 16) BK_MDG(16, 8);
    else if (k <= 24) BK_MDG(24, 4);
    else BK_MDG(32, 4);
#undef BK_MDG
}
static void launch_multiaxpy_burst(bk_ctx* ctx, int grid, size_t n, const double* V, size_t ldv, int k, const Coefs& cf, const double* src,
                                   double scale, double* dst, int want_norm, const double* dcoef, int gated) {
    int stag = 0;
    {
        const int P = (int)ctx->opt("axpy_stagger", 0.0);
        if (P > 1 && P < 256 && grid >= 2 * P)
            stag = P | (((int)ctx->opt("axpy_stagger_map", 0.0) & 255) << 8) | (((int)ctx->opt("axpy_stagger_units", 55.0) & 0x7fff) << 16);
    }
#define BK_MAC(KB)                                                                                                                                  \
    do {                                                                                                                                           \
        if (dcoef) hipLaunchKernelGGL((multiaxpy_c_kernel<KB, 4, true, true, true>), dim3(grid), dim3(kThreads), 0, ctx->stream, n, V, ldv, k, cf, src, scale, dst, want_norm, ctx->d_partials, dcoef, gated, stag); \
        else hipLaunchKernelGGL((multiaxpy_c_kernel<KB, 4, true, true, false>), dim3(grid), dim3(kThreads), 0, ctx->stream, n, V, ldv, k, cf, src, scale, dst, want_norm, ctx->d_partials, dcoef, gated, stag);     \
    } while (0)
    if (k <= 4) BK_MAC(4);
    else if (k <= 8) BK_MAC(8);
    else if (k <= 16) BK_MAC(16);
    else if (k <= 24) BK_MAC(24);
    else BK_MAC(32);
#undef BK_MAC
}

template <int KB>
static void launch_multidot(bk_ctx* ctx, bool vec, int grid, size_t n, const double* V, size_t ldv, int k, const double* w) {
    const unsigned xcd = xcd_map(ctx, n, grid, false, k);
    if (vec && nt_hint(ctx, n) && ctx->opt("dot_variant", 1.0) == 1.0) hipLaunchKernelGGL((multidot_kernel<KB, 2, true>), dim3(grid), dim3(kThreads), 0, ctx->stream, n, V, ldv, k, w, ctx->d_partials, (const double*)nullptr, xcd);
    else if (vec) hipLaunchKernelGGL((multidot_kernel<KB, 2>), dim3(grid), dim3(kThreads), 0, ctx->stream, n, V, ldv, k, w, ctx->d_partials);
    else hipLaunchKernelGGL((multidot_kernel<KB, 1>), dim3(grid), dim3(kThreads), 0, ctx->stream, n, V, ldv, k, w, ctx->d_partials);
}

int v_multidot(bk_ctx* ctx, size_t n, const double* V, size_t ldv, int k, const double* w, double* out) {
    if (k < 0 || k > kMaxBasis) return set_error(ctx, "v_multidot: k=%d out of range", k);
    const bool vec = aligned16(V) && aligned16(w) && (ldv % 2 == 0);
    const bool burst = burst_ok(ctx, vec, n, k);
    const int grid = burst ? burst_grid(ctx, n, "dot_blocks") : grid_for(n, vec ? 2 : 1, kRedBlocks);
    {
        ProfScope ps(ctx, "multidot", 8.0 * n * (k + 1));
        if (burst) launch_multidot_burst(ctx, grid, n, V, ldv, k, w, nullptr);
        else if (k <= 4) launch_multidot<4>(ctx, vec, grid, n, V, ldv, k, w);
        else if (k <= 8) launch_multidot<8>(ctx, vec, grid, n, V, ldv, k, w);
        else if (k <= 16) launch_multidot<16>(ctx, vec, grid, n, V, ldv, k, w);
        else if (k <= 24) launch_multidot<24>(ctx, vec, grid, n, V, ldv, k, w);
        else if (k <= 32) launch_multidot<32>(ctx, vec, grid, n, V, ldv, k, w);
        else if (k <= 48) launch_multidot<48>(ctx, vec, grid, n, V, ldv, k, w);
        else launch_multidot<64>(ctx, vec, grid, n, V, ldv, k, w);
        BK_HIP(ctx, hipGetLastError());
    }
    BK_TRY(reduce_finish(ctx, grid, k + 1, 0));
    for (int j = 0; j <= k; ++j) out[j] = ctx->h_red[j];
    return 0;
}

bool v_multidot_gram_ok(bk_ctx* ctx, size_t n, const double* V, size_t ldv, int k, const double* w) {
    return k >= 1 && k <= 2 * kBurstMax && n >= 2 && aligned16(V) && aligned16(w) && (ldv % 2 == 0) && ctx->opt("gmres_gram", 1.0) != 0.0;
}
int v_multidot_gram(bk_ctx* ctx, size_t n, const double* V, size_t ldv, int k, const double* w, double* out, double* gram) {
    const int grid = nt_hint(ctx, n) ? burst_grid(ctx, n, "dot_blocks") : grid_for(n, 2 * 4, 512);
    if (k <= kBurstMax) {
        {
            ProfScope ps(ctx, "multidot", 8.0 * n * (k + 1));
            launch_multidot_gram(ctx, grid, n, V, ldv, k, w, nullptr);
            BK_HIP(ctx, hipGetLastError());
        }
        BK_TRY(reduce_finish(ctx, grid, 2 * k + 1, 0));
        for (int j = 0; j <= k; ++j) out[j] = ctx->h_red[j];
        for (int j = 0; j < k; ++j) gram[j] = ctx->h_red[k + 1 + j];
        return 0;
    }
    const int k0 = kBurstMax, k1 = k - kBurstMax;
    {
        ProfScope ps(ctx, "multidot", 8.0 * n * (k0 + 2));
        launch_multidot_gram(ctx, grid, n, V, ldv, k0, w, nullptr, V + (size_t)(k - 1) * ldv);
        BK_HIP(ctx, hipGetLastError());
    }
    BK_TRY(reduce_finish(ctx, grid, 2 * k0 + 1, 0));
    for (int j = 0; j < k0; ++j) { out[j] = ctx->h_red[j]; gram[j] = ctx->h_red[k0 + 1 + j]; }
    {
        ProfScope ps(ctx, "multidot", 8.0 * n * (k1 + 1));
        launch_multidot_gram(ctx, grid, n, V + (size_t)k0 * ldv, ldv, k1, w, nullptr);
        BK_HIP(ctx, hipGetLastError());
    }
    BK_TRY(reduce_finish(ctx, grid, 2 * k1 + 1, 0));
    for (int j = 0; j < k1; ++j) { out[k0 + j] = ctx->h_red[j]; gram[k0 + j] = ctx->h_red[k1 + 1 + j]; }
    out[k] = ctx->h_red[k1];
    return 0;
}

bool v_block_ok(bk_ctx* ctx, size_t n, const double* V, size_t ldv) { return n >= 2 && aligned16(V) && (ldv % 2 == 0); }
int v_block_dots(bk_ctx* ctx, size_t n, const double* V, size_t ldv, int kold, int r0, int nr, double* D, double* T) {
    if (kold < 0 || kold > kMaxBasis || nr < 1 || nr > sstep::kR) return set_error(ctx, "v_block_dots: bad sizes");
    const bool nt = nt_hint(ctx, n);
    const int grid = nt ? burst_grid(ctx, n, "dot_blocks") : grid_for(n, 2 * 2, 512);
    const double* Rv = V + (size_t)r0 * ldv;
    int done = 0;
    constexpr int NR5 = 5;
    if (nr <= NR5 && kold > 4 && ctx->opt("block_dots_nr5", 1.0) != 0.0) {
        const int kb = std::min(kold, 8);
        constexpr int NV = 8 * NR5 + NR5 * (NR5 + 1) / 2;
        static_assert(NV <= kPartialVals, "d_partials too small");
        {
            ProfScope ps(ctx, "multidot", 8.0 * n * (kb + nr));
            if (nt) hipLaunchKernelGGL((block_dots_kernel<8, true, 2, true, NR5>), dim3(grid), dim3(kThreads), 0, ctx->stream, n, V, ldv, kb, Rv, nr, ctx->d_partials);
            else hipLaunchKernelGGL((block_dots_kernel<8, true, 2, false, NR5>), dim3(grid), dim3(kThreads), 0, ctx->stream, n, V, ldv, kb, Rv, nr, ctx->d_partials);
            BK_HIP(ctx, hipGetLastError());
        }
        BK_TRY(reduce_finish(ctx, grid, NV, 0));
        for (int i = 0; i < kb; ++i)
            for (int r = 0; r < sstep::kR; ++r) D[i * sstep::kR + r] = r < NR5 ? ctx->h_red[i * NR5 + r] : 0.0;
        for (int t = 0; t < sstep::kTri; ++t) T[t] = 0.0;
        for (int r = 0, t = 0; r < NR5; ++r)
            for (int c = r; c < NR5; ++c, ++t) T[sstep::tri(r, c)] = ctx->h_red[8 * NR5 + t];
        done = kb;
    } else {
        const int kb = std::min(kold, 4);
        {
            ProfScope ps(ctx, "multidot", 8.0 * n * (kb + nr));
            if (nt) hipLaunchKernelGGL((block_dots_kernel<4, true, 2, true>), dim3(grid), dim3(kThreads), 0, ctx->stream, n, V, ldv, kb, Rv, nr, ctx->d_partials);
            else hipLaunchKernelGGL((block_dots_kernel<4, true, 2, false>), dim3(grid), dim3(kThreads), 0, ctx->stream, n, V, ldv, kb, Rv, nr, ctx->d_partials);
            BK_HIP(ctx, hipGetLastError());
        }
        constexpr int NV = 4 * sstep::kR + sstep::kTri;
        static_assert(NV <= kPartialVals && 8 * sstep::kR <= kPartialVals && kMaxBasis + 2 <= kPartialVals, "d_partials too small");
        BK_TRY(reduce_finish(ctx, grid, NV, 0));
        for (int i = 0; i < kb; ++i)
            for (int r = 0; r < sstep::kR; ++r) D[i * sstep::kR + r] = ctx->h_red[i * sstep::kR + r];
        for (int t = 0; t < sstep::kTri; ++t) T[t] = ctx->h_red[4 * sstep::kR + t];
        done = kb;
    }
    for (int i0 = done; i0 < kold; i0 += 8) {
        const int kb = std::min(kold - i0, 8);
        {
            ProfScope ps(ctx, "multidot", 8.0 * n * (kb + nr));
            if (nt) hipLaunchKernelGGL((block_dots_kernel<8, false, 2, true>), dim3(grid), dim3(kThreads), 0, ctx->stream, n, V + (size_t)i0 * ldv, ldv, kb, Rv, nr, ctx->d_partials);
            else hipLaunchKernelGGL((block_dots_kernel<8, false, 2, false>), dim3(grid), dim3(kThreads), 0, ctx->stream, n, V + (size_t)i0 * ldv, ldv, kb, Rv, nr, ctx->d_partials);
            BK_HIP(ctx, hipGetLastError());
        }
        BK_TRY(reduce_finish(ctx, grid, 8 * sstep::kR, 0));
        for (int i = 0; i < kb; ++i)
            for (int r = 0; r < sstep::kR; ++r) D[(i0 + i) * sstep::kR + r] = ctx->h_red[i * sstep::kR + r];
    }
    return 0;
}

int v_block_axpy(bk_ctx* ctx, size_t n, double* V, size_t ldv, int k, int s, const double* Cm, const double* Tm) {
    if (k < 1 || k > 32 || s < 1 || s > sstep::kS) return set_error(ctx, "v_block_axpy: bad sizes");
    BlockCoefs cf;
    for (int i = 0; i < 32; ++i)
        for (int q = 0; q < sstep::kS; ++q) cf.c[i][q] = i < k ? Cm[i * sstep::kS + q] : 0.0;
    for (int r = 0; r < sstep::kS; ++r)
        for (int q = 0; q < sstep::kS; ++q) cf.t[r][q] = Tm[r * sstep::kS + q];
    const bool nt = nt_hint(ctx, n);
    const int grid = nt ? burst_grid(ctx, n, "axpy_burst_blocks") : grid_for(n, 2 * 2, 1024);
    double* Pv = V + (size_t)k * ldv;
    ProfScope ps(ctx, "multiaxpy", 8.0 * n * (k + 2 * s));
#define BK_BAX(KB)                                                                                                                          \
    do {                                                                                                                                    \
        if (nt) hipLaunchKernelGGL((block_axpy_kernel<KB, 4, true>), dim3(grid), dim3(kThreads), 0, ctx->stream, n, V, ldv, k, Pv, s, cf);   \
        else hipLaunchKernelGGL((block_axpy_kernel<KB, 4, false>), dim3(grid), dim3(kThreads), 0, ctx->stream, n, V, ldv, k, Pv, s, cf);     \
    } while (0)
    if (k <= 8) BK_BAX(8);
    else if (k <= 16) BK_BAX(16);
    else BK_BAX(32);
#undef BK_BAX
    BK_HIP(ctx, hipGetLastError());
    return 0;
}

template <int KB>
static void launch_multiaxpy(bk_ctx* ctx, bool vec, int grid, size_t n, const double* V, size_t ldv, int k, const Coefs& cf,
                             const double* src, double scale, double* dst, int want_norm) {
    const bool nt = ctx->opt("axpy_nt", 1.0) != 0.0;
    const int variant = nt_hint(ctx, n) ? (int)ctx->opt("axpy_variant", 3.0) : 0;
    const unsigned xcd = xcd_map(ctx, n, grid, true, k);
    if (vec && variant == 1) hipLaunchKernelGGL((multiaxpy_kernel<KB, 2, true, true, 1>), dim3(grid), dim3(kThreads), 0, ctx->stream, n, V, ldv, k, cf, src, scale, dst, want_norm, ctx->d_partials, xcd);
    else if (vec && variant == 2) hipLaunchKernelGGL((multiaxpy_kernel<KB, 2, true, false, 2>), dim3(grid), dim3(kThreads), 0, ctx->stream, n, V, ldv, k, cf, src, scale, dst, want_norm, ctx->d_partials, xcd);
    else if (vec && variant == 3) hipLaunchKernelGGL((multiaxpy_kernel<KB, 2, true, true, 2>), dim3(grid), dim3(kThreads), 0, ctx->stream, n, V, ldv, k, cf, src, scale, dst, want_norm, ctx->d_partials, xcd);
    else if (vec && nt) hipLaunchKernelGGL((multiaxpy_kernel<KB, 2, true>), dim3(grid), dim3(kThreads), 0, ctx->stream, n, V, ldv, k, cf, src, scale, dst, want_norm, ctx->d_partials);
    else if (vec) hipLaunchKernelGGL((multiaxpy_kernel<KB, 2>), dim3(grid), dim3(kThreads), 0, ctx->stream, n, V, ldv, k, cf, src, scale, dst, want_norm, ctx->d_partials);
    else hipLaunchKernelGGL((multiaxpy_kernel<KB, 1>), dim3(grid), dim3(kThreads), 0, ctx->stream, n, V, ldv, k, cf, src, scale, dst, want_norm, ctx->d_partials);
// ... 175 lines not shown
```

### bifurcationkit.jl_amd/hip.py

```python
from __future__ import annotations

import ctypes as C
import math
from dataclasses import dataclass, field

import numpy as np
import torch

from . import _lib as L


def _ptr(t):
    return C.c_void_p(t.data_ptr())


class Context:

    def __init__(self, device: int = 0, comm=None):
        if not torch.cuda.is_available():
            raise RuntimeError("bifurcationkit.jl_amd needs a visible MI355X (no CPU fallback)")
        self.lib = L.load()
        self.device = device
        torch.cuda.set_device(device)
        self.torch_device = torch.device("cuda", device)
# ... 795 lines not shown
        else:
            if self.ls is None:
                raise TypeError("EigArpack (HIP): the matrix-free shift-invert needs a linear solver `ls` for J - sigma I")
            if self.which != "LM":
                raise NotImplementedError("EigArpack (HIP): with sigma use which = :LM (eigenvalues closest to sigma)")
            core = ShiftInvert(self.sigma, self.ls, tol=max(self.tol, 10.0 * self.ls.rtol), maxiter=self.maxiter,
                               krylovdim=ncv, hermitian=self.hermitian, save_vectors=self.save_vectors, x0=self.v0)
        vals, vecs, cv, it = core(J, nev)
        return vals, vecs, True, 1

    @staticmethod
    def geteigenvector(vecs, n):
        return vecs[n]


@dataclass
class EigArnoldiMethod:
    sigma: float | None = None
    which: str = "LR"
    x0: object = None
    tol: float = 1.4901161193847656e-08
    maxdim: int | None = None
    restarts: int = 200
    hermitian: bool = False
    save_vectors: bool = True

    def __call__(self, J: HipJacobian, nev: int, **kwargs):
        if self.sigma is not None:
            import warnings
            warnings.warn("Shift-Invert strategy not implemented for maps")
        if self.which != "LR":
            raise NotImplementedError("EigArnoldiMethod (HIP): which = LR() only")
        maxdim = self.maxdim if self.maxdim is not None else max(20, 2 * nev)
        core = EigKrylovKit(tol=self.tol, maxiter=self.restarts, krylovdim=maxdim, hermitian=self.hermitian,
                            save_vectors=self.save_vectors, x0=self.x0)
        vals, vecs, cv, it = core(J, nev)
        return vals, vecs, cv, 1

    @staticmethod
    def geteigenvector(vecs, n):
        return vecs[n]


def newton_opts(tol, max_iterations, norm_inf, linesearch=False, alpha=1.0, alphamin=1e-3, callback=None):
    no = L.NewtonOpts()
    no.tol, no.max_iterations, no.norm_inf = float(tol), int(max_iterations), 1 if norm_inf else 0
    no.linesearch, no.alpha, no.alpha_min = 1 if linesearch else 0, float(alpha), float(alphamin)
    if callback is not None and hasattr(callback, "maxres"):
        no.max_residual = float(callback.maxres)
    elif callback is not None:
        def tramp(user, x, fx, residual, step, itlinear, p, z0u, z0p, from_newton):
            st = dict(x=x, residual=residual, step=step, itlinear=itlinear, p=p, z0=(z0u, z0p))
            st["fx" if from_newton else "res_f"] = fx
            try:
                return 1 if callback(st, fromNewton=bool(from_newton)) else 0
            except Exception:
                import traceback
                traceback.print_exc()
                return 0
        no.callback = L.NEWTON_CALLBACK(tramp)
        no._keepalive = (tramp, no.callback)
    return no


def newton_native(prob: _PdeProblem, x0: HipVec, p: float, ls: _GMRES, tol=1e-12, max_iterations=25, norm_inf=False,
                  callback=None):
    ctx = prob.ctx
    x = x0.copy()
    pv = prob._pvec(p)
    arr = (C.c_double * len(pv))(*pv)
    no = newton_opts(tol, max_iterations, norm_inf, callback=callback)
    lo = ls._opts()
    res = L.NewtonResult()
    ctx.check(ctx.lib.bk_newton(ctx.h, prob.h, _ptr(x.t), arr, len(pv), C.byref(no), C.byref(lo), ls._pl(),
                                C.byref(res)), "bk_newton")
    return dict(u=x, converged=bool(res.converged), itnewton=res.itnewton, itlineartot=res.itlinear,
                residuals=[res.residuals[i] for i in range(res.itnewton + 1)])


def newton_palc_native(prob: _PdeProblem, z0: BorderedArray, tau: BorderedArray, z_pred: BorderedArray, ds, theta,
                       bls: BorderingBLS, tol=1e-12, max_iterations=25, p_min=-math.inf, p_max=math.inf,
                       norm_inf=False, linesearch=False, alpha=1.0, alphamin=1e-3, callback=None):
    ctx = prob.ctx
    x = z_pred.u.copy()
    p = C.c_double(z_pred.p)
    pv = prob._pvec(z_pred.p)
    arr = (C.c_double * len(pv))(*pv)
    no = newton_opts(tol, max_iterations, norm_inf, linesearch, alpha, alphamin, callback)
    if isinstance(bls, MatrixFreeBLS):
        bo = L.BorderingOpts(0.0, 0, 1, 1)
    else:
        bo = L.BorderingOpts(bls.tol, 1 if bls.check_precision else 0, bls.k, 0)
    lo = bls.solver._opts()
    res = L.NewtonResult()
    big = 1.7e308
    ctx.check(ctx.lib.bk_newton_palc(
        ctx.h, prob.h, _ptr(x.t), C.byref(p), _ptr(z0.u.t), float(z0.p), _ptr(tau.u.t), float(tau.p), float(ds),
        float(theta), arr, len(pv), prob.ipar, max(float(p_min), -big), min(float(p_max), big), C.byref(no),
        C.byref(bo), C.byref(lo), bls.solver._pl(), C.byref(res)), "bk_newton_palc")
    return dict(u=BorderedArray(x, p.value), converged=bool(res.converged), itnewton=res.itnewton,
                itlineartot=res.itlinear, residuals=[res.residuals[i] for i in range(res.itnewton + 1)])


@dataclass
class DeflationOperator:
    power: float
    alpha: float
    roots: list = field(default_factory=list)
    accumulator: str = "prod"
    delta: float = 1e-8
    autodiff: bool = False

    def push(self, v):
        self.roots.append(v)

    def __len__(self):
        return len(self.roots)

    def dots(self, u: HipVec, du: HipVec = None):
        k = len(self.roots)
        ctx = u.ctx
        rp = (C.c_void_p * max(k, 1))(*[r.t.data_ptr() for r in self.roots])
        d = (C.c_double * max(k, 1))()
        e = (C.c_double * max(k, 1))() if du is not None else None
        ctx.check(ctx.lib.bk_deflation_dots(ctx.h, u.n, _ptr(u.t), _ptr(du.t) if du is not None else None, rp, k, d, e),
                  "bk_deflation_dots")
        return [d[i] for i in range(k)], (None if e is None else [e[i] for i in range(k)])

    def dist(self, u: HipVec):
        k = len(self.roots)
        ctx = u.ctx
        rp = (C.c_void_p * max(k, 1))(*[r.t.data_ptr() for r in self.roots])
        d2, dinf = (C.c_double * max(k, 1))(), (C.c_double * max(k, 1))()
        ctx.check(ctx.lib.bk_deflation_dist(ctx.h, u.n, _ptr(u.t), rp, k, d2, dinf), "bk_deflation_dist")
        return [d2[i] for i in range(k)], [dinf[i] for i in range(k)]

    def combine(self, d, e=None):
        k = len(d)
        if k == 0:
            return 1.0, 0.0
        mean = self.accumulator == "mean"
        power = float(self.power)
        inv = lambda x, q: math.inf if x == 0.0 else x ** q
        m = [(math.inf if di == 0.0 else 1.0 / di ** power) + self.alpha for di in d]
        acc = m[0]
        for mi in m[1:]:
            acc = acc + mi if mean else acc * mi
        M = acc / k if mean else acc
        if e is None:
            return M, None
        suf = [1.0] * (k + 1)
        for i in range(k - 1, -1, -1):
            suf[i] = m[i] * suf[i + 1]
        pre, s = 1.0, 0.0
        for i in range(k):
            g = (-2.0 * power * inv(d[i], -power - 1.0)) * e[i]
            s += g if mean else (pre * suf[i + 1]) * g
            pre *= m[i]
        return M, (s / k if mean else s)

    def __call__(self, u: HipVec) -> float:
        if not self.roots:
            return 1.0
        if self.autodiff:
            return self.combine(self.dots(u)[0])[0]
        out = None
        for r in self.roots:
            d = u.copy().add_(r, -1.0)
            m = 1.0 / d.inner(d) ** self.power + self.alpha
            out = m if out is None else (out * m if self.accumulator == "prod" else out + m)
        return out / len(self.roots) if self.accumulator == "mean" else out

    def dM(self, u: HipVec, du: HipVec) -> float:
        if not self.roots:
            return 0.0
        if self.autodiff:
            return self.combine(*self.dots(u, du))[1]
        return (self(u.copy().add_(du, self.delta)) - self(u)) / self.delta


def deflated_custom_ls(ls, prob, defop: DeflationOperator, u: HipVec, p, rhs: HipVec):
    Fu = prob.residual(u, p)
# ... 87 lines not shown
```

### include/bkhip.h

```cpp
#ifndef BKHIP_H
#define BKHIP_H

#include <stddef.h>

#ifdef __cplusplus
extern "C" {
#endif

typedef struct bk_ctx bk_ctx;
typedef struct bk_problem bk_problem;
typedef struct bk_op bk_op;
typedef struct bk_precond bk_precond;


#define BK_UNIQUE_ID_BYTES 128

int bk_version(void);
#define BK_ABI_VERSION 6
int bk_abi_version(void);
int bk_ctx_create(bk_ctx** ctx, int device, void* stream);
int bk_comm_unique_id(void* id128);
int bk_ctx_create_dist(bk_ctx** ctx, int device, void* stream, int rank, int nranks,
                       const void* id128);
typedef int (*bk_allreduce_fn)(void* user, double* buf, int n, int op);
// ... 97 lines not shown
typedef struct {
    double tol;
    int check_precision;
    int k;
    int kind;
} bk_bordering_opts;
int bk_bls_bordering(bk_ctx* ctx, bk_op* J, const double* dR, const double* dzu, double dzp,
                     const double* R, double n, double xiu, double xip, int has_shift,
                     double shift, double dotscale, const bk_bordering_opts* bopts,
                     const bk_gmres_opts* lsopts, bk_precond* pl, double* dX, double* dl,
                     int* converged, int itlinear[2]);
int bk_palc_update(bk_ctx* ctx, size_t n, double dl, const double* dx, const double* x1, double* x);
int bk_bls_matrixfree(bk_ctx* ctx, bk_op* J, const double* dR, const double* dzu, double dzp,
                      const double* R, double n, double xiu, double xip, int has_shift,
                      double shift, double dotscale, const bk_gmres_opts* lsopts, double* dX,
                      double* dl, int* converged, int* itlinear);

#define BK_MAX_BORDER 8
int bk_bls_block_bordering(bk_ctx* ctx, bk_op* J, int m, const double* const* b, const double* const* c,
                           const double* d, const double* rhst, const double* rhsb,
                           const bk_gmres_opts* lsopts, bk_precond* pl, double* u1, double* u2,
                           int* converged, int* itlinear);

int bk_bls_block_matrixfree(bk_ctx* ctx, bk_op* J, int m, const double* const* a, const double* const* b,
                            const double* c, const double* rhst, const double* rhsb, int has_shift,
                            double shift, double dotscale, const bk_gmres_opts* lsopts, double* u1,
                            double* u2, int* converged, int* itlinear);

int bk_bls_matrixfree_pl(bk_ctx* ctx, bk_op* J, const double* dR, const double* dzu, double dzp,
                         const double* R, double n, double xiu, double xip, int has_shift,
                         double shift, double dotscale, const bk_gmres_opts* lsopts, bk_precond* pl,
                         double* dX, double* dl, int* converged, int* itlinear);
int bk_bls_block_matrixfree_pl(bk_ctx* ctx, bk_op* J, int m, const double* const* a, const double* const* b,
                               const double* c, const double* rhst, const double* rhsb, int has_shift,
                               double shift, double dotscale, const bk_gmres_opts* lsopts, bk_precond* pl,
                               double* u1, double* u2, int* converged, int* itlinear);
int bk_bordered_tail(bk_ctx* ctx, size_t n, int m, double* y, const double* x, const double* const* atil,
                     const double* const* b, const double* coef, double* dots);

typedef struct {
    double sigma;
    int krylovdim;
    int maxiter;
    double tol;
    int hermitian;
    unsigned long long seed;
} bk_eig_opts;
int bk_eig_shiftinvert(bk_ctx* ctx, bk_op* J, int nev, const bk_eig_opts* eopts,
                       const bk_gmres_opts* lsopts, bk_precond* pl, double* vals_re,
                       double* vals_im, double* vecs, double* vecs_im, size_t ldvecs, int* nvals,
                       int* nconv, int* numops);
int bk_eig_set_start_vector(bk_ctx* ctx, const double* x0);
int bk_eig_krylovkit(bk_ctx* ctx, bk_op* J, int nev, const bk_eig_opts* eopts, double* vals_re, double* vals_im,
                     double* vecs, double* vecs_im, size_t ldvecs, int* nvals, int* nconv, int* numops);

typedef int (*bk_newton_callback)(void* user, const double* x, const double* fx, double residual, int step,
                                  int itlinear, double p, const double* z0u, double z0p, int from_newton);
typedef struct {
    double tol;
    int max_iterations;
    int norm_inf;
    int linesearch;
    double alpha;
    double alpha_min;
    double max_residual;
    bk_newton_callback callback;
    void* callback_user;
} bk_newton_opts;
#define BK_MAX_NEWTON_ITER 64
typedef struct {
    int converged;
    int itnewton;
    int itlinear;
    double residuals[BK_MAX_NEWTON_ITER + 1];
} bk_newton_result;
int bk_newton(bk_ctx* ctx, bk_problem* prob, double* x, const double* params, int nparams,
              const bk_newton_opts* nopts, const bk_gmres_opts* lsopts, bk_precond* pl,
              bk_newton_result* res);
int bk_newton_palc(bk_ctx* ctx, bk_problem* prob, double* x, double* p, const double* z0u,
                   double z0p, const double* tauu, double taup, double ds, double theta,
                   const double* params, int nparams, int ipar, double p_min, double p_max,
                   const bk_newton_opts* nopts, const bk_bordering_opts* bopts,
                   const bk_gmres_opts* lsopts, bk_precond* pl, bk_newton_result* res);

int bk_gmres_cshift(bk_ctx* ctx, bk_op* J, const double* rhs_re, const double* rhs_im, double* x_re,
                    double* x_im, double a0_re, double a0_im, double a1, const bk_gmres_opts* opts,
                    bk_precond* pl, int* converged, int* niter, double* resnorm);
int bk_bls_bordering_cshift(bk_ctx* ctx, bk_op* J, const double* dR_re, const double* dR_im,
                            const double* dzu_re, const double* dzu_im, double dzp_re, double dzp_im,
                            const double* R_re, const double* R_im, double n_re, double n_im, double xiu,
                            double xip, double shift_re, double shift_im, double dotscale,
                            const bk_gmres_opts* lsopts, bk_precond* pl, double* dX_re, double* dX_im,
                            double dl[2], int* converged, int itlinear[2]);
int bk_bls_matrixfree_pl_cshift(bk_ctx* ctx, bk_op* J, const double* dR_re, const double* dR_im,
                                const double* dzu_re, const double* dzu_im, double dzp_re, double dzp_im,
                                const double* R_re, const double* R_im, double n_re, double n_im, double xiu,
                                double xip, double shift_re, double shift_im, double dotscale,
                                const bk_gmres_opts* lsopts, bk_precond* pl, double* dX_re, double* dX_im,
                                double dl[2], int* converged, int* itlinear);
int bk_cbordered_tail(bk_ctx* ctx, size_t n, double* y_re, double* y_im, const double* x_re, const double* x_im,
                      const double* at_re, const double* at_im, const double* b_re, const double* b_im,
                      const double coef[2], double dots[2]);

#define BK_MAX_NEV 62
typedef struct {
    double ds, dsmin, dsmax;
    double a;
    double theta;
    double p_min, p_max;
    int tangent;
    int detect;
    int nev;
    double tol_stability;
} bk_cont_opts;
typedef struct {
    int converged, itnewton, itlinear;
    double residuals[BK_MAX_NEWTON_ITER + 1];
    double p;
    double ds_used, ds_next;
    int step;
    int stop;
    int n_unstable, n_imag, bifurcation;
    int nvals, eig_converged, eig_numops;
    double vals_re[BK_MAX_NEV + 1], vals_im[BK_MAX_NEV + 1];
    int tangent_converged;
    int natural;
} bk_cont_step_result;
typedef struct bk_cont bk_cont;
int bk_cont_create(bk_ctx* ctx, bk_problem* prob, const double* params, int nparams, int ipar,
                   const double* u0, double p0, const double* u1, double p1, const bk_cont_opts* copts,
                   const bk_newton_opts* nopts, const bk_bordering_opts* bopts, const bk_gmres_opts* lsopts,
                   bk_precond* pl, const bk_eig_opts* eopts, const bk_gmres_opts* eig_lsopts,
                   bk_precond* eig_pl, bk_cont_step_result* init, bk_cont** out);
int bk_cont_step(bk_cont* c, bk_cont_step_result* res);
int bk_cont_get(bk_cont* c, double* u, double* p, double* tauu, double* taup, double* ds);
int bk_cont_destroy(bk_cont* c);
int bk_cont_clone(bk_cont* src, bk_cont** out);
typedef struct {
    double dsmin_bisection;
    int n_inversion;
    int max_bisection_steps;
    double tol_bisection_eigenvalue;
    int max_steps;
} bk_bisection_opts;
typedef struct {
    int status, type;
    double interval[2];
    double p;
    int n_unstable[2], n_imag[2];
    int steps;
    int nvals;
    double vals_re[BK_MAX_NEV + 1], vals_im[BK_MAX_NEV + 1];
} bk_bisection_result;
int bk_cont_locate_bifurcation(bk_cont* c, const bk_bisection_opts* opts, bk_bisection_result* res);

int bk_newton_deflated(bk_ctx* ctx, bk_problem* prob, double* x, const double* params, int nparams,
                       const double* const* roots, int nroots, double power, double alpha,
                       int accumulator_mean, double delta, const bk_newton_opts* nopts,
                       const bk_gmres_opts* lsopts, bk_precond* pl, bk_newton_result* res);

int bk_deflation_dots(bk_ctx* ctx, size_t n, const double* u, const double* h ,
                      const double* const* roots, int nroots, double* d, double* e );
typedef struct {
    int converged;
    int itnewton;
    int itlinear;
// ... 187 lines not shown
```

Baseline: 11.61.

## Read PALC predictor in place, widen block dots, vectorize absmax reduction

Adds bk_newton_palc_from, which takes the predictor as a separate source. The first PALC update then reads from it directly instead of needing a full device copy into the work vector first, and the Python path allocates an uninitialised vector instead of copying. It also adds a specialised block-dots kernel for 6 right-hand vectors (previously handled by a slower fallback) and vectorises the inf-norm kernel with double2 loads and more per-thread work. The extra source pointer adds API surface, and the wide kernel uses more registers.

```diff
diff --git a/bifurcationkit.jl_amd/_lib.py b/bifurcationkit.jl_amd/_lib.py
--- a/bifurcationkit.jl_amd/_lib.py
+++ b/bifurcationkit.jl_amd/_lib.py
@@ -202,6 +202,9 @@
     "bk_newton_palc": (I, [VP, VP, VP, c_double_p, VP, D, VP, D, D, D, c_double_p, I, I, D, D,
                            C.POINTER(NewtonOpts), C.POINTER(BorderingOpts), C.POINTER(GmresOpts), VP,
                            C.POINTER(NewtonResult)]),
+    "bk_newton_palc_from": (I, [VP, VP, VP, VP, c_double_p, VP, D, VP, D, D, D, c_double_p, I, I, D, D,
+                                C.POINTER(NewtonOpts), C.POINTER(BorderingOpts), C.POINTER(GmresOpts), VP,
+                                C.POINTER(NewtonResult)]),
     "bk_d2f": (I, [VP, VP, c_double_p, I, VP, VP, VP]),
     "bk_djdp": (I, [VP, VP, c_double_p, I, I, VP, VP]),
     "bk_fold_contract": (I, [VP, VP, c_double_p, I, I, VP, VP, I, C.POINTER(VP), c_double_p]),
diff --git a/bifurcationkit.jl_amd/csrc/block_dots_body.h b/bifurcationkit.jl_amd/csrc/block_dots_body.h
--- /dev/null
+++ b/bifurcationkit.jl_amd/csrc/block_dots_body.h
@@ -0,0 +1,96 @@
+#pragma once
+#include "stream.h"
+
+namespace bk {
+namespace {
+
+template <int KB, bool TRI, int U, bool LDNT, int NRT>
+__device__ __forceinline__ void block_dots_body(size_t n, const double* __restrict__ V, size_t ldv, int kb,
+                                                const double* __restrict__ Rv, int nr, double* __restrict__ partials) {
+    constexpr int NR = NRT, NT3 = TRI ? NRT * (NRT + 1) / 2 : 1;
+    double acc[KB > 0 ? KB : 1][NR], tri[NT3];
+#pragma unroll
+    for (int i = 0; i < (KB > 0 ? KB : 1); ++i)
+#pragma unroll
+        for (int r = 0; r < NR; ++r) acc[i][r] = 0.0;
+#pragma unroll
+    for (int t = 0; t < NT3; ++t) tri[t] = 0.0;
+    stream_loop<U>(n >> 1, [&](auto uc, size_t i0, size_t st) {
+        constexpr int UU = decltype(uc)::value;
+        double2 rv[NR][UU];
+#pragma unroll
+        for (int r = 0; r < NR; ++r) {
+            if (r < nr) {
+#pragma unroll
+                for (int u = 0; u < UU; ++u) rv[r][u] = ld2<LDNT>(Rv + (size_t)r * ldv, i0 + u * st);
+            } else {
+#pragma unroll
+                for (int u = 0; u < UU; ++u) rv[r][u] = make_double2(0.0, 0.0);
+            }
+        }
+        if (TRI) {
+#pragma unroll
+            for (int r = 0; r < NR; ++r)
+#pragma unroll
+                for (int c = r; c < NR; ++c) {
+                    double a = tri[TRI ? r * NR - r * (r - 1) / 2 + (c - r) : 0];
+#pragma unroll
+                    for (int u = 0; u < UU; ++u) { a = fma(rv[r][u].x, rv[c][u].x, a); a = fma(rv[r][u].y, rv[c][u].y, a); }
+                    tri[TRI ? r * NR - r * (r - 1) / 2 + (c - r) : 0] = a;
+                }
+        }
+#pragma unroll
+        for (int i = 0; i < KB; ++i) {
+            if (i < kb) {
+                double2 vv[UU];
+#pragma unroll
+                for (int u = 0; u < UU; ++u) vv[u] = ld2<LDNT>(V + (size_t)i * ldv, i0 + u * st);
+#pragma unroll
+                for (int r = 0; r < NR; ++r)
+#pragma unroll
+                    for (int u = 0; u < UU; ++u) { acc[i][r] = fma(vv[u].x, rv[r][u].x, acc[i][r]); acc[i][r] = fma(vv[u].y, rv[r][u].y, acc[i][r]); }
+            }
+        }
+    });
+    if ((n & 1) && blockIdx.x == 0 && threadIdx.x == 0) {
+        double rl[NR];
+#pragma unroll
+        for (int r = 0; r < NR; ++r) rl[r] = r < nr ? Rv[(size_t)r * ldv + n - 1] : 0.0;
+        if (TRI) {
+#pragma unroll
+            for (int r = 0; r < NR; ++r)
+#pragma unroll
+                for (int c = r; c < NR; ++c) tri[TRI ? r * NR - r * (r - 1) / 2 + (c - r) : 0] = fma(rl[r], rl[c], tri[TRI ? r * NR - r * (r - 1) / 2 + (c - r) : 0]);
+        }
+#pragma unroll
+        for (int i = 0; i < KB; ++i)
+            if (i < kb) {
+                const double vl = V[(size_t)i * ldv + n - 1];
+#pragma unroll
+                for (int r = 0; r < NR; ++r) acc[i][r] = fma(vl, rl[r], acc[i][r]);
+            }
+    }
+    constexpr int NV = KB * NR + (TRI ? NR * (NR + 1) / 2 : 0);
+    __shared__ double sm[4][NV];
+    const int lane = threadIdx.x & 63, wid = threadIdx.x >> 6;
+#pragma unroll
+    for (int i = 0; i < KB; ++i)
+#pragma unroll
+        for (int r = 0; r < NR; ++r) {
+            const double s_ = wave_sum(acc[i][r]);
+            if (lane == 0) sm[wid][i * NR + r] = s_;
+        }
+    if (TRI) {
+#pragma unroll
+        for (int t = 0; t < NT3; ++t) {
+            const double s_ = wave_sum(tri[t]);
+            if (lane == 0) sm[wid][KB * NR + t] = s_;
+        }
+    }
+    __syncthreads();
+    for (int j = threadIdx.x; j < NV; j += kThreads)
+        partials[(size_t)blockIdx.x * NV + j] = (sm[0][j] + sm[1][j]) + (sm[2][j] + sm[3][j]);
+}
+
+}
+}
diff --git a/bifurcationkit.jl_amd/csrc/block_dots_wide.hip b/bifurcationkit.jl_amd/csrc/block_dots_wide.hip
--- /dev/null
+++ b/bifurcationkit.jl_amd/csrc/block_dots_wide.hip
@@ -0,0 +1,42 @@
+#include <algorithm>
+
+#include "block_dots_body.h"
+#include "common.h"
+#include "sstep.h"
+#include "stream.h"
+
+namespace bk {
+
+namespace {
+
+template <int KB, int U, bool LDNT, int NRT>
+__global__ void __launch_bounds__(kThreads) block_dots_wide_kernel(size_t n, const double* __restrict__ V, size_t ldv, int kb,
+                                                                   const double* __restrict__ Rv, int nr, double* __restrict__ partials) {
+    block_dots_body<KB, true, U, LDNT, NRT>(n, V, ldv, kb, Rv, nr, partials);
+}
+
+}
+
+int block_dots_wide(bk_ctx* ctx, int grid, bool nt, size_t n, const double* V, size_t ldv, int kold, const double* Rv, int nr,
+                    double* D, double* T, int* done) {
+    constexpr int NRW = kBlockDotsWideNr, NV = 8 * NRW + NRW * (NRW + 1) / 2;
+    static_assert(NV <= kPartialVals && NV <= kRedSlots && NRW <= sstep::kR, "d_partials / h_red too small");
+    if (nr < 1 || nr > NRW || kold < 1) return set_error(ctx, "block_dots_wide: bad sizes");
+    const int kb = std::min(kold, 8);
+    {
+        ProfScope ps(ctx, "multidot", 8.0 * n * (kb + nr));
+        if (nt) hipLaunchKernelGGL((block_dots_wide_kernel<8, 2, true, NRW>), dim3(grid), dim3(kThreads), 0, ctx->stream, n, V, ldv, kb, Rv, nr, ctx->d_partials);
+        else hipLaunchKernelGGL((block_dots_wide_kernel<8, 2, false, NRW>), dim3(grid), dim3(kThreads), 0, ctx->stream, n, V, ldv, kb, Rv, nr, ctx->d_partials);
+        BK_HIP(ctx, hipGetLastError());
+    }
+    BK_TRY(reduce_finish(ctx, grid, NV, 0));
+    for (int i = 0; i < kb; ++i)
+        for (int r = 0; r < sstep::kR; ++r) D[i * sstep::kR + r] = r < NRW ? ctx->h_red[i * NRW + r] : 0.0;
+    for (int t = 0; t < sstep::kTri; ++t) T[t] = 0.0;
+    for (int r = 0, t = 0; r < NRW; ++r)
+        for (int c = r; c < NRW; ++c, ++t) T[sstep::tri(r, c)] = ctx->h_red[8 * NRW + t];
+    *done = kb;
+    return 0;
+}
+
+}
diff --git a/bifurcationkit.jl_amd/csrc/common.h b/bifurcationkit.jl_amd/csrc/common.h
--- a/bifurcationkit.jl_amd/csrc/common.h
+++ b/bifurcationkit.jl_amd/csrc/common.h
@@ -204,6 +204,9 @@
 bool v_block_ok(bk_ctx* ctx, size_t n, const double* V, size_t ldv);
 int v_block_dots(bk_ctx* ctx, size_t n, const double* V, size_t ldv, int kold, int r0, int nr, double* D, double* T);
 int v_block_axpy(bk_ctx* ctx, size_t n, double* V, size_t ldv, int k, int s, const double* Cm, const double* Tm);
+constexpr int kBlockDotsWideNr = 6;
+int block_dots_wide(bk_ctx* ctx, int grid, bool nt, size_t n, const double* V, size_t ldv, int kold, const double* Rv, int nr,
+                    double* D, double* T, int* done);
 int v_arnoldi_step_dev(bk_ctx* ctx, size_t n, double* V, size_t ldv, int k, const double* w, double eta, double orth_tol,
                        double* rec, double* coef, double* gram = nullptr);
 int v_basis_combine(bk_ctx* ctx, size_t n, const double* V, size_t ldv, int m, const double* Qhost, int kout,
diff --git a/bifurcationkit.jl_amd/csrc/cont.hip b/bifurcationkit.jl_amd/csrc/cont.hip
--- a/bifurcationkit.jl_amd/csrc/cont.hip
+++ b/bifurcationkit.jl_amd/csrc/cont.hip
@@ -206,7 +206,6 @@
         return 0;
     }
     double* x = c->work;
-    BK_TRY(v_copy(ctx, c->n, c->predu, x));
     double p = c->predp;
     bk_newton_result nr = {};
     if (c->predp <= c->co.p_min || c->predp >= c->co.p_max) {
@@ -214,11 +213,12 @@
         double par[BK_MAX_PARAMS];
         for (int i = 0; i < c->nparams; ++i) par[i] = c->params[i];
         par[c->ipar] = p;
+        BK_TRY(v_copy(ctx, c->n, c->predu, x));
         BK_TRY(bk_newton(ctx, c->prob, x, par, c->nparams, &c->no, &c->lo, c->pl, &nr));
         r->natural = 1;
     } else {
-        BK_TRY(bk_newton_palc(ctx, c->prob, x, &p, c->zu, c->zp, c->tauu, c->taup, c->ds, c->co.theta, c->params,
-                              c->nparams, c->ipar, c->co.p_min, c->co.p_max, &c->no, &c->bo, &c->lo, c->pl, &nr));
+        BK_TRY(bk_newton_palc_from(ctx, c->prob, c->predu, x, &p, c->zu, c->zp, c->tauu, c->taup, c->ds, c->co.theta, c->params,
+                                   c->nparams, c->ipar, c->co.p_min, c->co.p_max, &c->no, &c->bo, &c->lo, c->pl, &nr));
     }
     r->converged = nr.converged; r->itnewton = nr.itnewton; r->itlinear = nr.itlinear;
     c->converged = nr.converged != 0;
diff --git a/bifurcationkit.jl_amd/csrc/ops.h b/bifurcationkit.jl_amd/csrc/ops.h
--- a/bifurcationkit.jl_amd/csrc/ops.h
+++ b/bifurcationkit.jl_amd/csrc/ops.h
@@ -199,7 +199,7 @@
 int bls_bordering(bk_ctx* ctx, bk_op* J, const double* dR, const double* dzu, double dzp, const double* R, double nn,
                   double xiu, double xip, bool has_shift, double shift, double dotscale, const bk_bordering_opts& bo,
                   const bk_gmres_opts& ls, bk_precond* pl, double* dX, double* dl, int* converged, int itlinear[2],
-                  double* xnew = nullptr);
+                  double* xnew = nullptr, const double* xsrc = nullptr);
 struct PrecOpView {
     bk_op* op = nullptr;
     bool tmode = false;
diff --git a/bifurcationkit.jl_amd/csrc/solver.hip b/bifurcationkit.jl_amd/csrc/solver.hip
--- a/bifurcationkit.jl_amd/csrc/solver.hip
+++ b/bifurcationkit.jl_amd/csrc/solver.hip
@@ -1113,7 +1113,7 @@
 
 template <int VEC, bool NTH>
 __global__ void __launch_bounds__(kThreads) palc_update_kernel(size_t n, double a, const double* __restrict__ dx,
-                                                               const double* __restrict__ x1, double* x, int has_dx) {
+                                                               const double* __restrict__ x1, const double* xs, double* x, int has_dx) {
     auto one = [&](double d, double v, double xv) {
         double t = 0.0;
         if (has_dx) t = __dmul_rn(a, d);
@@ -1128,7 +1128,7 @@
             for (int u = 0; u < UU; ++u) {
                 dv[u] = ld2<NTH>(dx, i0 + u * st);
                 vv[u] = ld2<NTH>(x1, i0 + u * st);
-                xv[u] = ld2<NTH>(x, i0 + u * st);
+                xv[u] = ld2<NTH>(xs, i0 + u * st);
             }
 #pragma unroll
             for (int u = 0; u < UU; ++u) {
@@ -1141,34 +1141,35 @@
                 }
             }
         });
-        if ((n & 1) && blockIdx.x == 0 && threadIdx.x == 0) x[n - 1] = one(dx[n - 1], x1[n - 1], x[n - 1]);
+        if ((n & 1) && blockIdx.x == 0 && threadIdx.x == 0) x[n - 1] = one(dx[n - 1], x1[n - 1], xs[n - 1]);
     } else {
-        for (size_t i = (size_t)blockIdx.x * kThreads + threadIdx.x; i < n; i += (size_t)gridDim.x * kThreads) x[i] = one(dx[i], x1[i], x[i]);
-    }
-}
-
-}
-
-int palc_update(bk_ctx* ctx, size_t n, double dl, const double* dx, const double* x1, double* x) {
+        for (size_t i = (size_t)blockIdx.x * kThreads + threadIdx.x; i < n; i += (size_t)gridDim.x * kThreads) x[i] = one(dx[i], x1[i], xs[i]);
+    }
+}
+
+}
+
+int palc_update(bk_ctx* ctx, size_t n, double dl, const double* dx, const double* x1, const double* xs, double* x) {
     if (n == 0) return 0;
     ProfScope ps(ctx, "blas1", 32.0 * n);
-    const bool vec = aligned16(dx) && aligned16(x1) && aligned16(x);
+    const bool vec = aligned16(dx) && aligned16(x1) && aligned16(xs) && aligned16(x);
     const int grid = grid_for(n, vec ? 2 : 1, 4096);
     const double a = -dl;
     const int has_dx = a != 0.0 ? 1 : 0;
     if (vec && nt_hint(ctx, n))
-        hipLaunchKernelGGL((palc_update_kernel<2, true>), dim3(grid), dim3(kThreads), 0, ctx->stream, n, a, dx, x1, x, has_dx);
+        hipLaunchKernelGGL((palc_update_kernel<2, true>), dim3(grid), dim3(kThreads), 0, ctx->stream, n, a, dx, x1, xs, x, has_dx);
     else if (vec)
-        hipLaunchKernelGGL((palc_update_kernel<2, false>), dim3(grid), dim3(kThreads), 0, ctx->stream, n, a, dx, x1, x, has_dx);
+        hipLaunchKernelGGL((palc_update_kernel<2, false>), dim3(grid), dim3(kThreads), 0, ctx->stream, n, a, dx, x1, xs, x, has_dx);
     else
-        hipLaunchKernelGGL((palc_update_kernel<1, false>), dim3(grid), dim3(kThreads), 0, ctx->stream, n, a, dx, x1, x, has_dx);
+        hipLaunchKernelGGL((palc_update_kernel<1, false>), dim3(grid), dim3(kThreads), 0, ctx->stream, n, a, dx, x1, xs, x, has_dx);
     BK_HIP(ctx, hipGetLastError());
     return 0;
 }
 
 static int bec(bk_ctx* ctx, bk_op* J, const double* dR, const double* dzu, double dzp, const double* R, double nn,
                double xiu, double xip, bool has_shift, double shift, double dotscale, const bk_gmres_opts& ls,
-               bk_precond* pl, BorderingState& st, double* x1, double* dl, int* cv, int it[2], double* xnew = nullptr) {
+               bk_precond* pl, BorderingState& st, double* x1, double* dl, int* cv, int it[2], double* xnew = nullptr,
+               const double* xsrc = nullptr) {
     const size_t n = J->n;
     GmresResult r1;
     const double a0 = has_shift ? shift : 0.0;
@@ -1183,7 +1184,7 @@
     BK_TRY(v_dot2(ctx, n, dzu, x1, st.dx, d));
     d[0] *= dotscale; d[1] *= dotscale;
     *dl = (nn - d[0] * xiu) / (dzp * xip - d[1] * xiu);
-    if (xnew) BK_TRY(palc_update(ctx, n, *dl, st.dx, x1, xnew));
+    if (xnew) BK_TRY(palc_update(ctx, n, *dl, st.dx, x1, xsrc ? xsrc : xnew, xnew));
     else BK_TRY(v_axpby(ctx, n, -(*dl), st.dx, 1.0, x1));
     *cv = r1.converged & st.cv_dx;
     it[0] = r1.niter; it[1] = st.it_dx;
@@ -1193,14 +1194,14 @@
 int bls_bordering(bk_ctx* ctx, bk_op* J, const double* dR, const double* dzu, double dzp, const double* R, double nn,
                   double xiu, double xip, bool has_shift, double shift, double dotscale, const bk_bordering_opts& bo,
                   const bk_gmres_opts& ls, bk_precond* pl, double* dX, double* dl, int* converged, int itlinear[2],
-                  double* xnew) {
+                  double* xnew, const double* xsrc) {
     if (xnew && bo.check_precision) return set_error(ctx, "bls_bordering: the fused update needs check_precision off");
     const size_t n = J->n;
     WsGuard ws(ctx);
     BorderingState st;
     BK_TRY(ws.get(n, &st.dx));
     int cv = 0, it[2] = {0, 0};
-    BK_TRY(bec(ctx, J, dR, dzu, dzp, R, nn, xiu, xip, has_shift, shift, dotscale, ls, pl, st, dX, dl, &cv, it, xnew));
+    BK_TRY(bec(ctx, J, dR, dzu, dzp, R, nn, xiu, xip, has_shift, shift, dotscale, ls, pl, st, dX, dl, &cv, it, xnew, xsrc));
     int k = 0;
     bool fail = true;
     double *dXr = nullptr, *dX1 = nullptr;
@@ -1284,7 +1285,7 @@
 int bk_palc_update(bk_ctx* ctx, size_t n, double dl, const double* dx, const double* x1, double* x) {
     if (!ctx || !dx || !x1 || !x) return -1;
     if (x == dx || x == x1) return set_error(ctx, "bk_palc_update: x must not alias dx or x1");
-    return palc_update(ctx, n, dl, dx, x1, x);
+    return palc_update(ctx, n, dl, dx, x1, x, x);
 }
 
 int bk_bls_matrixfree(bk_ctx* ctx, bk_op* J, const double* dR, const double* dzu, double dzp, const double* R,
@@ -1382,6 +1383,13 @@
     if (no->max_residual > 0.0 && !(residual < no->max_residual)) return 0;
     if (no->callback) return no->callback(no->callback_user, x, fx, residual, step, itlinear, p, z0u, z0p, from_newton) != 0;
     return 1;
+}
+
+static int palc_entry_copy(bk_ctx* ctx, size_t n, const double* x0, double* x) {
+    if (n == 0) return 0;
+    ProfScope ps(ctx, "entry_copy", 16.0 * n);
+    BK_HIP(ctx, hipMemcpyAsync(x, x0, n * sizeof(double), hipMemcpyDeviceToDevice, ctx->stream));
+    return 0;
 }
 
 }
@@ -1428,7 +1436,15 @@
                    const double* tauu, double taup, double ds, double theta, const double* params, int nparams,
                    int ipar, double p_min, double p_max, const bk_newton_opts* no, const bk_bordering_opts* bo,
                    const bk_gmres_opts* lsopts, bk_precond* pl, bk_newton_result* res) {
-    if (!ctx || !prob || !x || !p || !z0u || !tauu || !params || !no || !bo || !lsopts || !res) return -1;
+    return bk_newton_palc_from(ctx, prob, x, x, p, z0u, z0p, tauu, taup, ds, theta, params, nparams, ipar, p_min, p_max, no, bo,
+                               lsopts, pl, res);
+}
+
+int bk_newton_palc_from(bk_ctx* ctx, bk_problem* prob, const double* x0, double* x, double* p, const double* z0u, double z0p,
+                        const double* tauu, double taup, double ds, double theta, const double* params, int nparams,
+                        int ipar, double p_min, double p_max, const bk_newton_opts* no, const bk_bordering_opts* bo,
+                        const bk_gmres_opts* lsopts, bk_precond* pl, bk_newton_result* res) {
+    if (!ctx || !prob || !x0 || !x || !p || !z0u || !tauu || !params || !no || !bo || !lsopts || !res) return -1;
     if (ipar < 0 || ipar >= nparams || nparams > BK_MAX_PARAMS) return set_error(ctx, "bad parameter index");
     if (no->max_iterations > BK_MAX_NEWTON_ITER) return set_error(ctx, "max_iterations > %d", BK_MAX_NEWTON_ITER);
     const size_t n = prob->nloc;
@@ -1458,23 +1474,28 @@
         *out = (d * dotscale * theta + (pp - z0p) * taup * (1.0 - theta) - ds) - (dz0 * dotscale * theta);
         return 0;
     };
+    const bool fuse_update = bo->kind == 0 && bo->check_precision == 0 && !linesearch && ctx->opt("palc_fuse_update", 1.0) != 0.0;
+    const double* cur = x;
+    if (x0 != x) {
+        if (fuse_update && ctx->opt("palc_entry_copy", 0.0) == 0.0) cur = x0;
+        else BK_TRY(palc_entry_copy(ctx, n, x0, x));
+    }
     double pc = *p;
     par[ipar] = pc;
-    BK_TRY(bk_residual(prob, x, par, nparams, res_f));
+    BK_TRY(bk_residual(prob, cur, par, nparams, res_f));
     double res_n, rf;
-    BK_TRY(Nfun(x, pc, &res_n));
+    BK_TRY(Nfun(cur, pc, &res_n));
     BK_TRY(norm_of(ctx, n, res_f, inf, &rf));
     double r = std::max(rf, std::fabs(res_n));
     int step = 0, itlin = 0;
     res->residuals[0] = r;
     bool line_step = true;
-    const bool fuse_update = bo->kind == 0 && bo->check_precision == 0 && !linesearch && ctx->opt("palc_fuse_update", 1.0) != 0.0;
-    int compute = newton_cb(no, x, res_f, r, 0, 0, pc, z0u, z0p, 0);
+    int compute = newton_cb(no, cur, res_f, r, 0, 0, pc, z0u, z0p, 0);
     while (step < no->max_iterations && r > no->tol && line_step && compute) {
         par[ipar] = pc;
-        BK_TRY(prob->dparam(x, par, nparams, ipar, eps, res_f, dFdp));
+        BK_TRY(prob->dparam(cur, par, nparams, ipar, eps, res_f, dFdp));
         bk_op* J = nullptr;
-        BK_TRY(bk_jacobian(prob, x, par, nparams, &J));
+        BK_TRY(bk_jacobian(prob, cur, par, nparams, &J));
         double up = 0.0;
         int cv = 0, it[2] = {0, 0};
         int s;
@@ -1484,10 +1505,11 @@
             it[0] = itm; it[1] = 0;
         } else {
             s = bls_bordering(ctx, J, dFdp, tauu, taup, res_f, res_n, theta, 1.0 - theta, false, 0.0, dotscale, *bo,
-                              *lsopts, pl, u, &up, &cv, it, fuse_update ? x : nullptr);
+                              *lsopts, pl, u, &up, &cv, it, fuse_update ? x : nullptr, cur);
         }
         bk_op_destroy(J);
         if (s != 0) return s;
+        cur = x;
         itlin += it[0] + it[1];
         if (linesearch) {
             line_step = false;
@@ -1523,6 +1545,7 @@
         res->residuals[step] = r;
         compute = newton_cb(no, x, res_f, r, step, it[0] + it[1], pc, z0u, z0p, 0);
     }
+    if (cur != x) BK_TRY(palc_entry_copy(ctx, n, x0, x));
     *p = pc;
     res->converged = (res->residuals[step] < no->tol) & newton_cb(no, x, res_f, r, step, 0, pc, z0u, z0p, 0);
     res->itnewton = step;
diff --git a/bifurcationkit.jl_amd/csrc/vecops.hip b/bifurcationkit.jl_amd/csrc/vecops.hip
--- a/bifurcationkit.jl_amd/csrc/vecops.hip
+++ b/bifurcationkit.jl_amd/csrc/vecops.hip
@@ -1,6 +1,7 @@
 #include <algorithm>
 #include <type_traits>
 
+#include "block_dots_body.h"
 #include "common.h"
 #include "sstep.h"
 #include "stream.h"
@@ -282,11 +283,30 @@
     }
 }
 
+template <bool NTH>
+__device__ __forceinline__ double absmax_items(const double* __restrict__ xa, size_t n2) {
+    double m = 0.0;
+    stream_loop<4>(n2, [&](auto uc, size_t i0, size_t st) {
+        constexpr int UU = decltype(uc)::value;
+        double2 v[UU];
+#pragma unroll
+        for (int u = 0; u < UU; ++u) v[u] = ld2<NTH>(xa, i0 + u * st);
+#pragma unroll
+        for (int u = 0; u < UU; ++u) { m = max_nan(m, fabs(v[u].x)); m = max_nan(m, fabs(v[u].y)); }
+    });
+    return m;
+}
+
 __global__ void __launch_bounds__(kThreads) absmax_kernel(size_t n, const double* __restrict__ x,
                                                           double* __restrict__ partials) {
-    const size_t stride = (size_t)gridDim.x * kThreads;
-    double m = 0.0;
-    for (size_t i = (size_t)blockIdx.x * kThreads + threadIdx.x; i < n; i += stride) m = max_nan(m, fabs(x[i]));
+    const size_t head = (n > 0 && ((uintptr_t)x & 15) != 0) ? 1 : 0;
+    const double* xa = x + head;
+    const size_t rest = n - head;
+    double m = n >= ((size_t)1 << 22) ? absmax_items<true>(xa, rest >> 1) : absmax_items<false>(xa, rest >> 1);
+    if (blockIdx.x == 0 && threadIdx.x == 0) {
+        if (head) m = max_nan(m, fabs(x[0]));
+        if (rest & 1) m = max_nan(m, fabs(x[n - 1]));
+    }
     __shared__ double sm[4];
     m = wave_max(m);
     if ((threadIdx.x & 63) == 0) sm[threadIdx.x >> 6] = m;
@@ -578,89 +598,7 @@
 template <int KB, bool TRI, int U, bool LDNT, int NRT = sstep::kR>
 __global__ void __launch_bounds__(kThreads) block_dots_kernel(size_t n, const double* __restrict__ V, size_t ldv, int kb,
                                                               const double* __restrict__ Rv, int nr, double* __restrict__ partials) {
-    constexpr int NR = NRT, NT3 = TRI ? NRT * (NRT + 1) / 2 : 1;
-    double acc[KB > 0 ? KB : 1][NR], tri[NT3];
-#pragma unroll
-    for (int i = 0; i < (KB > 0 ? KB : 1); ++i)
-#pragma unroll
-        for (int r = 0; r < NR; ++r) acc[i][r] = 0.0;
-#pragma unroll
-    for (int t = 0; t < NT3; ++t) tri[t] = 0.0;
-    stream_loop<U>(n >> 1, [&](auto uc, size_t i0, size_t st) {
-        constexpr int UU = decltype(uc)::value;
-        double2 rv[NR][UU];
-#pragma unroll
-        for (int r = 0; r < NR; ++r) {
-            if (r < nr) {
-#pragma unroll
-                for (int u = 0; u < UU; ++u) rv[r][u] = ld2<LDNT>(Rv + (size_t)r * ldv, i0 + u * st);
-            } else {
-#pragma unroll
-                for (int u = 0; u < UU; ++u) rv[r][u] = make_double2(0.0, 0.0);
-            }
-        }
-        if (TRI) {
-#pragma unroll
-            for (int r = 0; r < NR; ++r)
-#pragma unroll
-                for (int c = r; c < NR; ++c) {
-                    double a = tri[TRI ? r * NR - r * (r - 1) / 2 + (c - r) : 0];
-#pragma unroll
-                    for (int u = 0; u < UU; ++u) { a = fma(rv[r][u].x, rv[c][u].x, a); a = fma(rv[r][u].y, rv[c][u].y, a); }
-                    tri[TRI ? r * NR - r * (r - 1) / 2 + (c - r) : 0] = a;
-                }
-        }
-#pragma unroll
-        for (int i = 0; i < KB; ++i) {
-            if (i < kb) {
-                double2 vv[UU];
-#pragma unroll
-                for (int u = 0; u < UU; ++u) vv[u] = ld2<LDNT>(V + (size_t)i * ldv, i0 + u * st);
-#pragma unroll
-                for (int r = 0; r < NR; ++r)
-#pragma unroll
-                    for (int u = 0; u < UU; ++u) { acc[i][r] = fma(vv[u].x, rv[r][u].x, acc[i][r]); acc[i][r] = fma(vv[u].y, rv[r][u].y, acc[i][r]); }
-            }
-        }
-    });
-    if ((n & 1) && blockIdx.x == 0 && threadIdx.x == 0) {
-        double rl[NR];
-#pragma unroll
-        for (int r = 0; r < NR; ++r) rl[r] = r < nr ? Rv[(size_t)r * ldv + n - 1] : 0.0;
-        if (TRI) {
-#pragma unroll
-            for (int r = 0; r < NR; ++r)
-#pragma unroll
-                for (int c = r; c < NR; ++c) tri[TRI ? r * NR - r * (r - 1) / 2 + (c - r) : 0] = fma(rl[r], rl[c], tri[TRI ? r * NR - r * (r - 1) / 2 + (c - r) : 0]);
-        }
-#pragma unroll
-        for (int i = 0; i < KB; ++i)
-            if (i < kb) {
-                const double vl = V[(size_t)i * ldv + n - 1];
-#pragma unroll
-                for (int r = 0; r < NR; ++r) acc[i][r] = fma(vl, rl[r], acc[i][r]);
-            }
-    }
-    constexpr int NV = KB * NR + (TRI ? NR * (NR + 1) / 2 : 0);
-    __shared__ double sm[4][NV];
-    const int lane = threadIdx.x & 63, wid = threadIdx.x >> 6;
-#pragma unroll
-    for (int i = 0; i < KB; ++i)
-#pragma unroll
-        for (int r = 0; r < NR; ++r) {
-            const double s_ = wave_sum(acc[i][r]);
-            if (lane == 0) sm[wid][i * NR + r] = s_;
-        }
-    if (TRI) {
-#pragma unroll
-        for (int t = 0; t < NT3; ++t) {
-            const double s_ = wave_sum(tri[t]);
-            if (lane == 0) sm[wid][KB * NR + t] = s_;
-        }
-    }
-    __syncthreads();
-    for (int j = threadIdx.x; j < NV; j += kThreads)
-        partials[(size_t)blockIdx.x * NV + j] = (sm[0][j] + sm[1][j]) + (sm[2][j] + sm[3][j]);
+    block_dots_body<KB, TRI, U, LDNT, NRT>(n, V, ldv, kb, Rv, nr, partials);
 }
 
 struct BlockCoefs {
@@ -1017,7 +955,7 @@
 }
 
 int v_nrminf(bk_ctx* ctx, size_t n, const double* x, double* out) {
-    const int grid = grid_for(n, 1, kRedBlocks);
+    const int grid = grid_for(n, 2 * 4, kRedBlocks);
     {
         ProfScope ps(ctx, "blas1", 8.0 * n);
         hipLaunchKernelGGL(absmax_kernel, dim3(grid), dim3(kThreads), 0, ctx->stream, n, x, ctx->d_partials);
@@ -1159,7 +1097,9 @@
     const double* Rv = V + (size_t)r0 * ldv;
     int done = 0;
     constexpr int NR5 = 5;
-    if (nr <= NR5 && kold > 4 && ctx->opt("block_dots_nr5", 1.0) != 0.0) {
+    if (nr > NR5 && nr <= kBlockDotsWideNr && kold > 4 && ctx->opt("block_dots_wide", 1.0) != 0.0) {
+        BK_TRY(block_dots_wide(ctx, grid, nt, n, V, ldv, kold, Rv, nr, D, T, &done));
+    } else if (nr <= NR5 && kold > 4 && ctx->opt("block_dots_nr5", 1.0) != 0.0) {
         const int kb = std::min(kold, 8);
         constexpr int NV = 8 * NR5 + NR5 * (NR5 + 1) / 2;
         static_assert(NV <= kPartialVals, "d_partials too small");
diff --git a/bifurcationkit.jl_amd/hip.py b/bifurcationkit.jl_amd/hip.py
--- a/bifurcationkit.jl_amd/hip.py
+++ b/bifurcationkit.jl_amd/hip.py
@@ -901,7 +901,7 @@
                        bls: BorderingBLS, tol=1e-12, max_iterations=25, p_min=-math.inf, p_max=math.inf,
                        norm_inf=False, linesearch=False, alpha=1.0, alphamin=1e-3, callback=None):
     ctx = prob.ctx
-    x = z_pred.u.copy()
+    x = z_pred.u.similar()
     p = C.c_double(z_pred.p)
     pv = prob._pvec(z_pred.p)
     arr = (C.c_double * len(pv))(*pv)
@@ -913,10 +913,10 @@
     lo = bls.solver._opts()
     res = L.NewtonResult()
     big = 1.7e308
-    ctx.check(ctx.lib.bk_newton_palc(
-        ctx.h, prob.h, _ptr(x.t), C.byref(p), _ptr(z0.u.t), float(z0.p), _ptr(tau.u.t), float(tau.p), float(ds),
+    ctx.check(ctx.lib.bk_newton_palc_from(
+        ctx.h, prob.h, _ptr(z_pred.u.t), _ptr(x.t), C.byref(p), _ptr(z0.u.t), float(z0.p), _ptr(tau.u.t), float(tau.p), float(ds),
         float(theta), arr, len(pv), prob.ipar, max(float(p_min), -big), min(float(p_max), big), C.byref(no),
-        C.byref(bo), C.byref(lo), bls.solver._pl(), C.byref(res)), "bk_newton_palc")
+        C.byref(bo), C.byref(lo), bls.solver._pl(), C.byref(res)), "bk_newton_palc_from")
     return dict(u=BorderedArray(x, p.value), converged=bool(res.converged), itnewton=res.itnewton,
                 itlineartot=res.itlinear, residuals=[res.residuals[i] for i in range(res.itnewton + 1)])
 
diff --git a/include/bkhip.h b/include/bkhip.h
--- a/include/bkhip.h
+++ b/include/bkhip.h
@@ -203,6 +203,11 @@
                    const double* params, int nparams, int ipar, double p_min, double p_max,
                    const bk_newton_opts* nopts, const bk_bordering_opts* bopts,
                    const bk_gmres_opts* lsopts, bk_precond* pl, bk_newton_result* res);
+int bk_newton_palc_from(bk_ctx* ctx, bk_problem* prob, const double* x0, double* x, double* p,
+                        const double* z0u, double z0p, const double* tauu, double taup, double ds,
+                        double theta, const double* params, int nparams, int ipar, double p_min,
+                        double p_max, const bk_newton_opts* nopts, const bk_bordering_opts* bopts,
+                        const bk_gmres_opts* lsopts, bk_precond* pl, bk_newton_result* res);
 
 int bk_gmres_cshift(bk_ctx* ctx, bk_op* J, const double* rhs_re, const double* rhs_im, double* x_re,
                     double* x_im, double a0_re, double a0_im, double a1, const bk_gmres_opts* opts,
```

New measurement: 11.81, median of 6. 1.02x the previous value.
